# zhipeng-wei/Image-to-Video-I2V-attack

Measured on AMD Instinct MI355X. Metric: adversarial frames/sec (10-step I2V, ResNet-50 layer3, 32x224^2 clips), higher is better.
Workload: dtype f32

## Files before the change

### __graft_entry__.py

```python
import os
import subprocess
import sys

ROOT = os.path.dirname(os.path.abspath(__file__))
PKG_ROOT = os.path.join(ROOT, "image-to-video-i2v-attack_amd")
CSRC = os.path.join(PKG_ROOT, "csrc")
LIB = os.path.join(PKG_ROOT, "i2v_amd", "libi2v_hip.so")
for p in (PKG_ROOT, ROOT):
    if p not in sys.path:
        sys.path.insert(0, p)


def _stale(target, sources):
    return not os.path.exists(target) or any(os.path.getmtime(s) > os.path.getmtime(target) for s in sources)


ENGINE_UNITS = ["i2v_engine.cpp", "i2v_pack.cpp", "i2v_plan.cpp", "i2v_tune.cpp", "i2v_run.cpp", "i2v_loop_api.cpp"]
UNITS = ["i2v_kernels.hip", "i2v_conv_cfg0.hip", "i2v_conv_cfg1.hip", "i2v_conv_cfg2.hip", "i2v_conv_cfg3.hip", "i2v_conv_cfg4.hip",
         "i2v_conv_cfg5.hip", "i2v_conv_scpair.hip", "i2v_conv_stems.hip", "i2v_fastblock.hip", "i2v_gconv.hip", "i2v_dwconv.hip", "i2v_se.hip", "i2v_loader.hip", "i2v_vit.hip", "i2v_vit.cpp", "i2v_swin.hip", "i2v_swin.cpp",
         "i2v_convnext.hip", "i2v_convnext.cpp", "i2v_mixer.hip", "i2v_mixer.cpp",
         ] + ENGINE_UNITS
HEADERS = ["i2v_kernels.h", "i2v_params.h", "i2v_be.h", "i2v_conv_tile.h", "i2v_conv_launch.h", "i2v_vit_kernels.h", "i2v_swin_kernels.h", "i2v_xf.h",
           "i2v_net.h", "i2v_se_host.h", "i2v_convnext_host.h", "i2v_xf_host.h", "i2v_hip_stub.h",
           "i2v_mixer_host.h", "i2v_gelu.h", "i2v_scpair_host.h"]
FLAGS = ["--offload-arch=gfx950", "-O3", "-ffp-contract=off", "-std=c++20", "-fPIC", "-DI2V_SEPARATE_UNITS",
         "-DI2V_HAVE_GCONV", "-DI2V_HAVE_DWCONV",
         "-DI2V_HAVE_SE",
         "-DI2V_HAVE_CONVNEXT",
         "-DI2V_HAVE_MIXER",
         "-DI2V_HAVE_SCPAIR"]


def build_lib(experimental: bool = False) -> str:
    from concurrent.futures import ThreadPoolExecutor
    hipcc = os.environ.get("HIPCC", "/opt/rocm/bin/hipcc")
    lib = LIB.replace(".so", "_exp.so") if experimental else LIB
    objdir = os.path.join(CSRC, "build", "exp" if experimental else "default")
    os.makedirs(objdir, exist_ok=True)
    units = UNITS + (["i2v_conv_exp.hip"] if experimental else [])
    hdrs = [os.path.join(CSRC, f) for f in HEADERS] + [os.path.join(ROOT, "include", h) for h in ("i2v_hip.h", "i2v_loader.h", "i2v_vit.h", "i2v_swin.h", "i2v_convnext.h", "i2v_mixer.h")]
    defs = ["-DI2V_EXPERIMENTAL"] if experimental else []
    if not _stale(lib, [os.path.join(CSRC, u) for u in units] + hdrs):
        return lib
    jobs = []
    for u in units:
        src, obj = os.path.join(CSRC, u), os.path.join(objdir, u + ".o")
        if _stale(obj, [src] + hdrs):
            jobs.append([hipcc] + FLAGS + defs + ["-c", "-x", "hip", src, "-o", obj])

    def run(cmd):
        print(" ".join(cmd), flush=True)
        subprocess.run(cmd, check=True)
    if jobs:
        with ThreadPoolExecutor(max_workers=min(len(jobs), max(1, (os.cpu_count() or 2)))) as ex:
            list(ex.map(run, jobs))
    objs = [os.path.join(objdir, u + ".o") for u in units]
    if jobs or _stale(lib, objs):
        run([hipcc, "--offload-arch=gfx950", "-shared", "-fPIC", "-o", lib] + objs)
    return lib


def build() -> None:
    build_lib(experimental=False)
    deps = [os.path.join(CSRC, f) for f in ENGINE_UNITS + ["i2v_net.h", "i2v_kernels.h", "i2v_params.h", "i2v_se_host.h", "i2v_convnext_host.h", "i2v_convnext.cpp", "i2v_mixer_host.h", "i2v_mixer.cpp", "i2v_scpair_host.h", "i2v_gelu.h", "i2v_xf.h", "i2v_xf_host.h", "i2v_hip_stub.h",
                                                               "i2v_vit_kernels.h", "i2v_swin_kernels.h"]] + [os.path.join(ROOT, "include", "i2v_hip.h")]
    hs = os.path.join(ROOT, "tests", "hostsim")
    if _stale(os.path.join(hs, "libi2v_hostsim.so"), deps + [os.path.join(hs, "hostsim_backend.cpp")]):
        subprocess.run([os.path.join(hs, "build.sh")], check=True)
    import ctypes
    import i2v_amd
    from i2v_amd import lib
    cd = ctypes.CDLL(LIB) if not _has_gpu() else lib.load()
    missing = [n for n in lib.EXPORTS + lib.LOADER_EXPORTS + lib.VIT_EXPORTS + lib.SWIN_EXPORTS + lib.CONVNEXT_EXPORTS + lib.MIXER_EXPORTS if not hasattr(cd, n)]
    if missing:
        raise RuntimeError(f"libi2v_hip.so lacks symbols: {missing}")


def _has_gpu() -> bool:
    try:
        import torch
        return torch.cuda.is_available()
    except Exception:
        return False


def smoke() -> None:
    import numpy as np
    import torch
    build()
    from i2v_amd import attacks, graphs, weights
    from oracle import restate
    gen = torch.Generator().manual_seed(1234)
    u8 = torch.randint(0, 256, (1, 3, 4, 64, 64), generator=gen, dtype=torch.uint8)
    mean = torch.tensor(restate.MEAN).view(1, 3, 1, 1, 1)
    std = torch.tensor(restate.STD).view(1, 3, 1, 1, 1)
    vid = (u8.float() / 255 - mean) / std
    atk = attacks.ImageGuidedFMDirection_Adam(["resnet"], depth=3, step_size=0.005, steps=3,
                                              graph_builder=graphs.build_tiny, weight_seed=0)
    adv = atk(vid, torch.zeros(1, dtype=torch.long), ["smoke"])
    torch.cuda.synchronize()
    g = graphs.build_tiny("resnet", (64, 64))
    net = restate.OracleNet(g, weights.synthetic_state_dict(g, 0), [g.hooks[3]])
    ref = restate.run_attack([net], vid, steps=3, step_size=0.005)
    np.testing.assert_allclose(atk.last_costs, ref["costs"], rtol=2e-4)
    diff = (adv.cpu() - ref["adv"]).abs()
    assert float(diff.mean()) < 5e-3, float(diff.mean())
    print("smoke ok: costs", atk.last_costs, "mean|adv-oracle|", float(diff.mean()))


if __name__ == "__main__":
    if "--experimental" in sys.argv[1:]:
        print(build_lib(experimental=True))
    else:
        build()
        if _has_gpu():
            smoke()
```

### image-to-video-i2v-attack_amd/csrc/i2v_be.h

```cpp
#pragma once
#include <hip/hip_runtime.h>
#include <math.h>
#include <stdint.h>
#include <stdio.h>
#include <stdlib.h>
#include <string.h>

#include <type_traits>
#include <utility>

#include "i2v_kernels.h"

typedef float f32x16 __attribute__((ext_vector_type(16)));
typedef float f32x4 __attribute__((ext_vector_type(4)));

extern thread_local char g_be_err[256];
extern thread_local bool g_be_has_err;
int hip_fail(hipError_t e, const char* what);
#define HIPCHK(x) do { hipError_t e_ = (x); if (e_ != hipSuccess) return hip_fail(e_, #x); } while (0)
#define LAUNCH_CHECK(name) do { hipError_t e_ = hipGetLastError(); if (e_ != hipSuccess) return hip_fail(e_, name); } while (0)
extern long long g_stat_conv, g_stat_pws, g_stat_bf3, g_stat_igh, g_stat_sth, g_stat_fastblock, g_stat_vfma, g_stat_igv, g_stat_gconv, g_stat_dwconv, g_stat_se, g_stat_cndw, g_stat_mixtok, g_stat_scpair;

__device__ __forceinline__ unsigned fastdiv(unsigned n, unsigned m, unsigned s) {
    return (unsigned)(((unsigned long long)n * m) >> s);
}
static inline void fastdiv_magic(unsigned d, uint32_t* m, uint32_t* s) {
    unsigned l = 0; while ((1ull << l) < d) ++l;
    *s = 31 + l;
    *m = (uint32_t)(((1ull << (31 + l)) / d) + 1);
}
typedef int i2v_v4i __attribute__((ext_vector_type(4)));
__device__ __forceinline__ I2VKEntry load_kentry(const I2VKEntry* tab, int k) {
#if defined(__HIP_DEVICE_COMPILE__)
    const i2v_v4i v = ((const __attribute__((address_space(4))) i2v_v4i*)tab)[k];
    return I2VKEntry{v.x, v.y, v.z, v.w};
#else
    return tab[k];
#endif
}

static inline void conv_magics(I2VConvParams& p) {
    fastdiv_magic((unsigned)(p.Hg * p.Wg), &p.dv_hw_m, &p.dv_hw_s);
    fastdiv_magic((unsigned)p.Wg, &p.dv_w_m, &p.dv_w_s);
    fastdiv_magic((unsigned)(p.Tg > 0 ? p.Tg : 1), &p.dv_t_m, &p.dv_t_s);
    fastdiv_magic((unsigned)(p.Wo > 0 ? p.Wo : 1), &p.dv_wo_m, &p.dv_wo_s);
}

static inline bool conv_wants_prefetch(const I2VConvParams& p) {
    return p.vec_epilogue && !p.gate_scale && !p.pre_scale && p.add0_stride == 1 && (p.add0 || p.add1 || p.mask || p.gate) && p.Kpad <= 256 && (p.pointwise || p.tap_uniform) && p.Cd > 32;
}

static inline int conv_tail_px_tiles(const I2VConvParams& p) {
    if (p.quad || p.pre_scale || p.temporal || !(p.pointwise || p.tap_uniform) || p.Cd % 16 != 0 || p.blk > 1) return 0;
    const int64_t P = (int64_t)p.N * p.Hg * p.Wg;
    const int64_t n_px = (P + 63) / 64; const int n_cd = (p.Cd + 63) / 64;
    const int64_t tiles = n_px * n_cd;
    if (tiles < 2 * 256) return 0;
    const int r = (int)(tiles % 256);
    if (r == 0 || r > 104) return 0;
    return r / n_cd;
}

static inline bool conv_halo_ok(const I2VConvParams& p) {
    return p.halo == 9 && p.tap_uniform && !p.temporal && !p.pre_scale && !p.quad && p.blk <= 1 && p.sh == 1 && p.sw == 1 && p.Hs == p.Hg &&
           p.Ws == p.Wg && (p.Ws == 14 || p.Ws == 28 || p.Ws == 56) && p.Kpad == p.K && (p.Kpad / I2V_KC) % 9 == 0;
}

static inline bool conv_dc_ok(const I2VConvParams& p) {
    return (p.pointwise || p.tap_uniform) && !p.temporal && !p.pre_scale && !p.quad && p.Cd > 32 && (p.Kpad / I2V_KC) % 2 == 0 && p.Kpad >= 4 * I2V_KC;
}

static inline bool conv_bf3_ok(const I2VConvParams& p) {
#ifdef I2V_EXPERIMENTAL
    return p.bf3 && p.wp3 && (p.pointwise || p.tap_uniform) && (!p.temporal || p.tap_uniform) && !p.pre_scale && !p.quad && p.blk <= 1 && p.blkt <= 1 && p.Cd > 32;
#else
    (void)p; return false;
#endif
}

int launch_conv_cfg0(const I2VConvParams& p, hipStream_t s);
int launch_conv_cfg1(const I2VConvParams& p, hipStream_t s);
int launch_conv_cfg2(const I2VConvParams& p, hipStream_t s);
int launch_conv_cfg3(const I2VConvParams& p, hipStream_t s);
int launch_conv_cfg4(const I2VConvParams& p, hipStream_t s);
int launch_conv_cfg5(const I2VConvParams& p, hipStream_t s);
bool conv_ighalo_ok(const I2VConvParams& p);
int launch_conv_ighalo(const I2VConvParams& p, hipStream_t s);
bool conv_igvfma_ok(const I2VConvParams& p);
int launch_conv_igvfma(const I2VConvParams& p, hipStream_t s);
bool conv_stemhalo_ok(const I2VConvParams& p);
int launch_conv_stemhalo(const I2VConvParams& p, hipStream_t s);
bool conv_vfma_ok(const I2VConvParams& p);
int launch_conv_vfma(const I2VConvParams& p, hipStream_t s);
#ifdef I2V_EXPERIMENTAL
#ifndef I2V_BF3_VARIANT
#define I2V_BF3_VARIANT 1
#endif
#endif
#ifdef I2V_EXPERIMENTAL
bool conv_stem64_ok(const I2VConvParams& p);
int launch_conv_stem64(const I2VConvParams& p, hipStream_t s);
int conv_pws_grid(const I2VConvParams& p);
int launch_conv_pws(const I2VConvParams& p, hipStream_t s);
int launch_conv_bf3(const I2VConvParams& p, hipStream_t s);
// ... 2 lines not shown
```

### image-to-video-i2v-attack_amd/csrc/i2v_conv_tile.h

```cpp
#pragma once
#include "i2v_be.h"

#ifndef I2V_PROBE_T
struct I2VNoProbe {
    __device__ __forceinline__ void entry() {}
    __device__ __forceinline__ void loop_begin() {}
    __device__ __forceinline__ void loop_end(int ) {}
    __device__ __forceinline__ void exit(int ) {}
};
#define I2V_PROBE_T I2VNoProbe
#endif

#ifndef I2V_PRIO_LEVELS
#define I2V_PRIO_LEVELS 3
#endif
#ifndef I2V_DEEP
#define I2V_DEEP 1
#endif
#ifndef I2V_DEEP_STAGES
#define I2V_DEEP_STAGES 3
#endif
#ifndef I2V_BF3_STAGES
#define I2V_BF3_STAGES 2
#endif
#ifndef I2V_SMALL_WPE
#define I2V_SMALL_WPE 7
#endif
#ifndef I2V_PREF_WPE
#define I2V_PREF_WPE 6
#endif
#ifndef I2V_MID_WPE
#define I2V_MID_WPE 5
#endif
#ifndef I2V_TALL_WPE
#define I2V_TALL_WPE 6
#endif
#ifndef I2V_BIG_WPE
#define I2V_BIG_WPE 3
#endif

static constexpr int conv_waves_per_simd(int BD, int BP, bool PREF, bool hi, int MODE = 0) {
    return (BD == 64 && BP == 64) ? (PREF ? (I2V_DEEP && MODE == 1 && I2V_DEEP_STAGES > 3 ? 4  : I2V_PREF_WPE) : I2V_SMALL_WPE) : (BD == 128 && BP == 64) ? I2V_TALL_WPE : (BD == 32 && BP == 256) ? 4  : BD * BP == 8192 ? I2V_MID_WPE : BD * BP == 16384 ? I2V_BIG_WPE : (hi ? 8 : 1);
}
#define I2V_CONV_WPE __attribute__((amdgpu_waves_per_eu(conv_waves_per_simd(BD, BP, PREF, false, MODE), conv_waves_per_simd(BD, BP, PREF, true, MODE))))
static constexpr bool conv_deep(int MODE, bool PREF) { return I2V_DEEP && PREF && MODE == 1; }
template <int BD, int BP, int WD, bool MF16, int NST = 2, int CPB = 1, int BF3 = 0>
constexpr int conv_lds_floats() {
    constexpr int stage = NST * CPB * (I2V_KC * BP + (BF3 == 2 ? 0 : BF3 ? ((BD / 32) * 3 + 3) / 4 * 4 * 256 : I2V_KC * BD)), epi = WD * (MF16 ? 16 : 32) * BP;
    return stage > epi ? stage : epi;
}

template <int HWM>
constexpr int conv_halo_lds_floats() {
    constexpr int stage = 2 * I2V_KC * (64 + 64 + 2 * HWM + 2), epi = 64 * 64;
    return stage > epi ? stage : epi;
}

template <int BD, int BP, int WD, bool PREF, bool MF16, bool FUSE, typename PT>
__device__ __forceinline__ void conv_vec_rows(const PT& p, const int i, const int cd0, const int64_t px0, const float (*const Cs)[BP], const int t,
                                              const float4* const pre0, const unsigned* const pregw, float* const mid) {
    constexpr int FR = MF16 ? 16 : 32;
    const int lane = t & 63;
    const int HWg = p.Hg * p.Wg, HoWo = p.Ho * p.Wo;
    const int64_t P = (int64_t)p.N * HWg;
    (void)pre0; (void)pregw; (void)mid;
#ifdef I2V_NT_ALL
    const bool nt_store = true;
#else
    const bool nt_store = p.cfg > 0 && ((p.cfg - 1) & 128);
#endif
    constexpr int C4 = BP / 4, RSTEP = 1024 / BP, NQ = WD * FR / RSTEP;
    const int c4 = t % C4, rbase = t / C4;
    const int64_t pp = px0 + (int64_t)c4 * 4;
    const bool pok = pp < P;
    const int64_t n = pok ? fastdiv((unsigned)pp, p.dv_hw_m, p.dv_hw_s) : 0;
    const int64_t poff = pp - n * HWg;
    #pragma unroll
    for (int q = 0; q < NQ; ++q) {
        const int row = rbase + q * RSTEP;
        const int cd = cd0 + (row / FR) * (BD / WD) + i * FR + (row % FR);
        const bool valid = pok && cd < p.Cd;
        float4 v = make_float4(0.f, 0.f, 0.f, 0.f);
        if (valid) {
        v = *reinterpret_cast<const float4*>(&Cs[row][c4 * 4]);
        const int64_t o = (int64_t)cd * HoWo + poff;
        if (p.gate_scale) {
            const float4 m = *reinterpret_cast<const float4*>(p.mask + n * p.mask_nstride + o);
            const float gs = p.gate_scale[cd], gt = p.gate_shift[cd];
            if (!(fmaf(m.x, gs, gt) > 0.f)) v.x = 0.f;
            if (!(fmaf(m.y, gs, gt) > 0.f)) v.y = 0.f;
            if (!(fmaf(m.z, gs, gt) > 0.f)) v.z = 0.f;
            if (!(fmaf(m.w, gs, gt) > 0.f)) v.w = 0.f;
        }
        if (p.shift) { const float sh = p.shift[cd]; v.x += sh; v.y += sh; v.z += sh; v.w += sh; }
        if (PREF) {
            v.x += pre0[q].x; v.y += pre0[q].y; v.z += pre0[q].z; v.w += pre0[q].w;
        } else {
            if (p.add0 && p.add0_stride == 1) {
                const float4 a = *reinterpret_cast<const float4*>(p.add0 + n * p.add0_nstride + o);
                v.x += a.x; v.y += a.y; v.z += a.z; v.w += a.w;
            } else if (p.add0) {
                const int oh = (int)fastdiv((unsigned)poff, p.dv_wo_m, p.dv_wo_s), ow = (int)(poff - (int64_t)oh * p.Wo);
                if (!(oh & 1) && (oh >> 1) < p.add0_H) {
                    const float2 a = *reinterpret_cast<const float2*>(
                        p.add0 + n * p.add0_nstride + (int64_t)cd * p.add0_H * p.add0_W + (oh >> 1) * p.add0_W + (ow >> 1));
                    v.x += a.x; v.z += a.y;
                }
            }
        }
        if (p.add1) {
            const float4 a = *reinterpret_cast<const float4*>(p.add1 + n * p.add1_nstride + o);
            v.x += a.x; v.y += a.y; v.z += a.z; v.w += a.w;
        }
        if (p.relu) { v.x = fmaxf(v.x, 0.f); v.y = fmaxf(v.y, 0.f); v.z = fmaxf(v.z, 0.f); v.w = fmaxf(v.w, 0.f); }
        if (p.gate) {
            const unsigned w = PREF ? pregw[q] : p.gate[(int64_t)cd * p.gate_stride + ((p.gate_pix0 + pp) >> 5)];
            const unsigned g = w >> ((unsigned)(p.gate_pix0 + pp) & 31u);
            if (!(g & 1u)) v.x = 0.f;
            if (!(g & 2u)) v.y = 0.f;
            if (!(g & 4u)) v.z = 0.f;
            if (!(g & 8u)) v.w = 0.f;
        } else if (p.mask && !p.gate_scale) {
            const float4 m = *reinterpret_cast<const float4*>(p.mask + n * p.mask_nstride + o);
            if (!(m.x > 0.f)) v.x = 0.f;
            if (!(m.y > 0.f)) v.y = 0.f;
            if (!(m.z > 0.f)) v.z = 0.f;
            if (!(m.w > 0.f)) v.w = 0.f;
        }
        if constexpr (!FUSE) {
            if (nt_store) { typedef float nt4 __attribute__((ext_vector_type(4))); const nt4 w4 = {v.x, v.y, v.z, v.w};
                            __builtin_nontemporal_store(w4, reinterpret_cast<nt4*>(p.dst + n * p.dst_nstride + o)); }
            else *reinterpret_cast<float4*>(p.dst + n * p.dst_nstride + o) = v;
        }
        }
        if constexpr (FUSE)
            *reinterpret_cast<float4*>(mid + (cd - cd0) * BP + c4 * 4) = v;
        if (p.gate_out) {
            unsigned nib = valid ? ((v.x > 0.f ? 1u : 0u) | (v.y > 0.f ? 2u : 0u) | (v.z > 0.f ? 4u : 0u) | (v.w > 0.f ? 8u : 0u)) : 0u;
            nib <<= 4 * (lane & 7);
            nib |= (unsigned)__builtin_amdgcn_update_dpp(0, (int)nib, 0xB1, 0xF, 0xF, true);
            nib |= (unsigned)__builtin_amdgcn_update_dpp(0, (int)nib, 0x4E, 0xF, 0xF, true);
            nib |= (unsigned)__builtin_amdgcn_update_dpp(0, (int)nib, 0x141, 0xF, 0xF, true);
            if (valid && (lane & 7) == 0)
                p.gate_out[(int64_t)cd * p.gate_out_stride + ((p.gate_out_pix0 + pp) >> 5)] = nib;
        }
    }
}

#define I2V_FROW(r) (MF16 ? 4 * lk + (r) : ((r) & 3) + 8 * ((r) >> 2) + 4 * lk)
template <int BP, int WP, bool MF16, int TP, typename ACC>
__device__ __forceinline__ void conv_acc_to_rows(ACC (&acc)[TP], float (*const Cs)[BP]) {
    constexpr int FR = MF16 ? 16 : 32, NR = MF16 ? 4 : 16;
    const int lane = threadIdx.x & 63, wave = threadIdx.x >> 6;
    const int wd = wave / WP, wpx = wave % WP;
    const int l31 = MF16 ? (lane & 15) : (lane & 31), lk = MF16 ? (lane >> 4) : (lane >> 5);
    __syncthreads();
#pragma unroll
    for (int j = 0; j < TP; ++j)
#pragma unroll
        for (int r = 0; r < NR; ++r)
            Cs[wd * FR + I2V_FROW(r)][wpx * (BP / WP) + j * FR + l31] = acc[j][r];
    __syncthreads();
}
template <int BD, int BP, int WD, int WP, bool PREF, bool MF16, bool FUSE, typename ACC, typename PT>
__device__ __forceinline__ void conv_vec_epilogue(const PT& p, ACC (&acc)[BD / WD / (MF16 ? 16 : 32)][BP / WP / (MF16 ? 16 : 32)], const int cd0,
                                                  const int64_t px0, float* const smem, const float4* const pre0, const unsigned* const pregw,
                                                  float* const mid) {
    constexpr int FR = MF16 ? 16 : 32, TD = BD / WD / FR;
    const int t = threadIdx.x;
    float (*Cs)[BP] = reinterpret_cast<float (*)[BP]>(smem);
#pragma unroll
    for (int i = 0; i < TD; ++i) {
        conv_acc_to_rows<BP, WP, MF16>(acc[i], Cs);
        conv_vec_rows<BD, BP, WD, PREF, MF16, FUSE>(p, i, cd0, px0, Cs, t, pre0, pregw, mid);
    }
}
#undef I2V_FROW

__device__ __forceinline__ int conv_xcd_lid(const int bid, const int nwg) {
    const int q8 = nwg >> 3, r8 = nwg & 7, xcd = bid & 7;
    return (xcd < r8 ? xcd * (q8 + 1) : r8 * (q8 + 1) + (xcd - r8) * q8) + (bid >> 3);
}

template <int BD, int BP, int WD, int WP, int MODE, bool PREF, bool PRE = false, bool VID = false, bool MF16 = false, int HWM = 0, int CPB = 1, int FUSE = 0, int BF3 = 0>
__device__ __forceinline__ void conv_tile_loop(const I2VConvParams& p, const int cd0, const int64_t px0, const int nwg, float* const smem, I2V_PROBE_T& probe,
                                               const int probe_slot, const int prio_arg,
                                               typename std::conditional<MF16, f32x4, f32x16>::type (&acc)[BD / WD / (MF16 ? 16 : 32)][BP / WP / (MF16 ? 16 : 32)],
                                               float4 (&pre0)[PREF ? WD * (MF16 ? 16 : 32) / (1024 / BP) : 1], unsigned (&pregw)[PREF ? WD * (MF16 ? 16 : 32) / (1024 / BP) : 1]) {
#if defined(__HIP_DEVICE_COMPILE__)
    constexpr int KC = I2V_KC;
    constexpr int FR = MF16 ? 16 : 32;
    constexpr int NR = MF16 ? 4 : 16;
    constexpr int TD = BD / WD / FR, TP = BP / WP / FR;
    static_assert(!(MF16 && (PRE || PREF)), "no pre-activation / prefetch variants of the 16x16 tile");
    constexpr bool DEEP = conv_deep(MODE, PREF) || (BF3 == 1 && I2V_BF3_STAGES > 2) || BF3 == 3;
    constexpr int NST = BF3 == 3 ? 3 : BF3 == 1 ? I2V_BF3_STAGES : DEEP ? I2V_DEEP_STAGES : 2, AHEAD = NST - 1;
    constexpr bool HALO = MODE == 5;
    constexpr int HS = HALO ? BP + 2 * HWM + 2 : 1, HQ = (HS + 63) / 64;
    static_assert(!HALO || (HWM > 0 && BD == 64 && BP == 64 && !PREF && !PRE && !VID && !MF16), "halo staging: the plain 64x64 image tile only");
    static_assert(CPB == 1 || (!HALO && !DEEP && !PREF && !PRE && MODE != 4 && MODE != 0), "several chunks per barrier: the plain pointwise / tap-uniform loops only");
    constexpr int KB = CPB * KC;
    static_assert(!BF3 || (!MF16 && !PRE && !PREF && !HALO && (MODE == 1 || MODE == 2) && FUSE == 0 && BD % 32 == 0), "split-bf16 K loop: the plain pointwise / tap-uniform tiles");
    constexpr int AF = BF3 == 2 ? 0 : BF3 ? CPB * (((BD / 32) * 3 + 3) / 4 * 4) * 256 : KB * BD;
    float (*As)[KB][BD] = reinterpret_cast<float (*)[KB][BD]>(smem);
    float* const As3 = smem;
    float (*Bs)[KB][BP] = reinterpret_cast<float (*)[KB][BP]>(smem + NST * AF);

    const int t = threadIdx.x, lane = t & 63, wave = t >> 6;
    const int wd = wave / WP, wpx = wave % WP;

    const int HWg = p.Hg * p.Wg;
    const int64_t P = (int64_t)p.N * HWg;

    constexpr bool PW = MODE == 1;
    constexpr bool QUAD = MODE == 4;
    typedef __attribute__((address_space(3))) void* lds_ptr_t;
    constexpr unsigned OOB = 0x80000000u;
    const int wv = __builtin_amdgcn_readfirstlane(wave);
    const __amdgpu_buffer_rsrc_t rs_w = BF3 ? __builtin_amdgcn_make_buffer_rsrc((void*)p.wp3, 0, (p.Kpad / KC) * (p.Cdpad / 32) * 3072, 0x00020000)
                                            : __builtin_amdgcn_make_buffer_rsrc((void*)p.wp, 0, p.Kpad * p.Cdpad * 4, 0x00020000);
    constexpr unsigned XB = QUAD ? 64u : 0u;
    const __amdgpu_buffer_rsrc_t rs_x = __builtin_amdgcn_make_buffer_rsrc((void*)((const char*)p.src - XB), 0, p.src_span_bytes + 2 * XB, 0x00020000);
    constexpr int NA = BF3 == 2 ? 0 : BF3 ? (BD / 32) * 3 : KC * BD / 256, NAQ = (NA + 3) / 4;
    constexpr int BPER = (PW || QUAD) ? 256 : 64;
    constexpr int NB = HALO ? 0 : KC * BP / BPER, NBQ = (NB + 3) / 4;
    const int bcol = PW ? (lane * 4) % BP : (BP >= 64 ? ((wave * 64) % BP) + lane : lane % BP);
    const int64_t ppix = px0 + bcol;
    const bool pvalid = ppix < P;
    const int64_t pn = pvalid ? fastdiv((unsigned)ppix, p.dv_hw_m, p.dv_hw_s) : 0;
    const int prem = (int)(ppix - pn * HWg);
    const int HWs = p.Hs * p.Ws;
    int h0 = 0, w0 = 0, t0 = 0;
    int64_t pns = pn;
    if (VID) {
        const int64_t clip = fastdiv((unsigned)pn, p.dv_t_m, p.dv_t_s);
        t0 = (int)(pn - clip * p.Tg) * p.st;
        pns = clip * p.Ts + t0;
    }
    const int nstr = (int)p.src_nstride;
    unsigned xoff;
    if (PW) xoff = (unsigned)((pns * p.src_nstride + prem) * 4);
    else {
        const int gi = (int)fastdiv((unsigned)prem, p.dv_w_m, p.dv_w_s), gj = prem - gi * p.Wg;
        h0 = gi * p.sh; w0 = gj * p.sw;
        xoff = (unsigned)((pns * p.src_nstride + (int64_t)h0 * p.Ws + w0) * 4) + XB;
    }
    if (!pvalid) xoff = OOB;
    unsigned aoff[NAQ ? NAQ : 1];
#pragma unroll
    for (int q = 0; q < NAQ; ++q) {
        const int f = (wave + 4 * q) * 256 + lane * 4;
        aoff[q] = BF3 ? (unsigned)(((cd0 / 32) * 3 + wave + 4 * q) * 1024 + lane * 16) : (unsigned)(((f / BD) * p.Cdpad + f % BD + cd0) * 4);
    }
    unsigned boff[PW ? NBQ : 1];
    if (PW) {
#pragma unroll
        for (int q = 0; q < NBQ; ++q) boff[q] = pvalid ? xoff + (unsigned)((((wave + 4 * q) * 256 + lane * 4) / BP) * HWs * 4) : OOB;
// ... 670 lines not shown
```

### image-to-video-i2v-attack_amd/csrc/i2v_engine.cpp

```cpp
#include "i2v_net.h"

#include <math.h>
#include <stdarg.h>
#include <stdio.h>
#include <stdlib.h>
#include <string.h>

using namespace eng;

#define I2V_MAX_NETS 4096
thread_local std::string eng::g_err;

int eng::fail(const char* fmt, ...) {
    char buf[512];
    va_list ap;
    va_start(ap, fmt);
    vsnprintf(buf, sizeof buf, fmt, ap);
    va_end(ap);
    g_err = buf;
    return 1;
}

int i2v_api_fail(const char* msg) { return fail("%s", msg); }

// ... 343 lines not shown
        if (nd.groups > 1 || nd.dw) std::vector<float>().swap(nd.w);
    }
    size_t off = 64;
    for (const Node& nd : n.nodes) if (nd.type == 0 && nd.cd.src == n.input && nd.fwd.quad) n.stage_input = true;
    if (n.stage_input) {
        const Buffer& ib = n.bufs[n.tens[n.input].buf];
        n.in_stage_off = off; off = align_up(off + N * ib.C * ib.H * ib.W, 64) + 64;
    }
    for (Buffer& b : n.bufs) {
        if (b.is_input) continue;
        size_t sz = N / Tin * b.T * b.C * b.H * b.W;
        b.act_off = off; off = align_up(off + sz, 64);
        b.grad_off = off; off = align_up(off + sz, 64);
    }
    const char* gates_env = getenv("I2V_GATES");
    const bool use_gates = !(gates_env && gates_env[0] == '0');
    for (const Node& nd : n.nodes)
        if (use_gates && nd.type == 0 && nd.cd.relu && !nd.fwd.tpair) n.bufs[n.tens[nd.cd.dst].buf].gated = true;
    for (const Node& nd : n.nodes)
        if (use_gates && nd.type == 4 && nd.sd.relu) n.bufs[n.tens[nd.sd.dst].buf].gated = true;
    for (Buffer& b : n.bufs) {
        if (!b.gated) continue;
        const size_t pix = N / Tin * b.T * b.H * b.W;
        if (pix + 64 >= (1ull << 31)) return fail("gate rows of more than 2^31 bits are not supported");
        b.gate_words = (int)((pix + 31) / 32 + 2);
        b.gate_off = off; off = align_up(off + (size_t)b.C * b.gate_words, 64);
    }
    for (Node& nd : n.nodes)
        if (nd.type == 1) {
            const Buffer& db = n.bufs[n.tens[nd.pd.dst].buf];
            nd.idx_off = off; off = align_up(off + (N / Tin * db.T * n.tens[nd.pd.dst].C * db.H * db.W + 3) / 4, 64);
        }
    for (Node& nd : n.nodes)
        if (nd.type == 3) {
            const Buffer& tb = n.bufs[n.tens[nd.ad.theta].buf]; const Buffer& pb = n.bufs[n.tens[nd.ad.phi].buf];
            nd.p_off = off; off = align_up(off + N / Tin * ((size_t)tb.T * tb.H * tb.W) * ((size_t)pb.T * pb.H * pb.W), 64);
        }
    for (Node& nd : n.nodes)
        if (nd.type == 4) {
            const size_t C = (size_t)nd.sd.C, rd = (size_t)nd.sd.rd;
            nd.se_off = off; nd.se_floats = 4 * align_up(N * C, 64) + align_up(N * rd, 64);
            off += nd.se_floats;
        }
    std::string err;
    size_t end = 0;
    if (!plan_pass(n, true, off, N, &end, &err)) return fail("plan: %s", err.c_str());
    n.arena_floats = end + 64;
    n.arena = (float*)be_malloc(n.arena_floats * sizeof(float));
    if (!n.arena) return fail("arena allocation of %zu bytes failed", n.arena_floats * sizeof(float));
    CHECK_BE(be_memset0(n.arena, n.arena_floats * sizeof(float), nullptr));
    if (!plan_pass(n, false, off, N, &end, &err)) return fail("plan: %s", err.c_str());
    mark_fusable(n);
    if (autotune(n)) return 1;
    mark_overlap(n);
    CHECK_BE(be_stream_sync(nullptr));
    n.planned = true;
    return 0;
}

extern "C" int i2v_net_fusion_info(i2v_handle h, int net, int32_t out[4]) {
    Net* n = get_net(h, net); if (!n) return 1;
    if (!n->planned || !out) return fail("i2v_net_fusion_info: net not planned");
    out[0] = out[1] = out[2] = out[3] = 0;
    int k = 0;
    for (const std::vector<Launch>* L : {&n->fwd, &n->bwd}) {
        for (const Launch& l : *L) { out[k] += l.fuse_ok ? 1 : 0; out[2 + k] += (l.fuse_ok && l.fuse_b[0]) ? 1 : 0; }
        ++k;
    }
    return 0;
}

extern "C" int i2v_net_scpair_info(i2v_handle h, int net, int32_t out[4]) {
    Net* n = get_net(h, net); if (!n) return 1;
    if (!n->planned || !out) return fail("i2v_net_scpair_info: net not planned");
    out[0] = out[1] = out[2] = out[3] = 0;
    int k = 0;
    for (const std::vector<Launch>* L : {&n->fwd, &n->bwd}) {
        for (const Launch& l : *L) { out[k] += l.sc_ok ? 1 : 0; out[2 + k] += (l.sc_ok && l.sc_b[0]) ? 1 : 0; }
        ++k;
    }
    return 0;
}

extern "C" size_t i2v_net_workspace_bytes(i2v_handle h, int net) {
    Net* n = get_net(h, net); if (!n) return 0;
    return n->arena_floats * sizeof(float) + n->weight_bytes;
}

#ifndef I2V_SEPARATE_UNITS
#include "i2v_pack.cpp"
#include "i2v_plan.cpp"
#include "i2v_tune.cpp"
#include "i2v_run.cpp"
#include "i2v_loop_api.cpp"
#define fail xf_fail
#include "i2v_convnext.cpp"
#include "i2v_mixer.cpp"
#undef fail
#endif
```

### image-to-video-i2v-attack_amd/csrc/i2v_kernels.h

```cpp
#pragma once
#include <initializer_list>
#include "i2v_params.h"

typedef void* i2v_stream_t;

const char* be_name();
long long be_stat(const char* name);
int  be_set_device(int device);
void* be_malloc(size_t bytes);
void be_free(void* p);
int  be_h2d(void* dst, const void* src, size_t bytes);
int  be_d2d_2d(void* dst, size_t dpitch, const void* src, size_t spitch, size_t width, size_t rows,
               i2v_stream_t s);
int  be_memset0(void* p, size_t bytes, i2v_stream_t s);
const char* be_error();
int  i2v_api_fail(const char* msg);
void* be_event_create();
void be_event_destroy(void* ev);
int  be_event_record(void* ev, i2v_stream_t s);
int  be_event_elapsed_ms(void* start, void* stop, float* ms);
int  be_stream_sync(i2v_stream_t s);
i2v_stream_t be_stream_create();
void be_stream_destroy(i2v_stream_t s);
int  be_stream_wait_event(i2v_stream_t s, void* ev);
int  be_device_sync();

int k_conv(const I2VConvParams& p, i2v_stream_t s);
int k_conv_fusable(const I2VConvParams& a, const I2VConvParams& b);
inline bool i2v_conv_pair_fusable(const I2VConvParams& a, const I2VConvParams& b) {
    if (a.pointwise || !a.tap_uniform || a.temporal || a.quad || a.pre_scale || a.gate_scale || a.blk > 1 || a.blkt > 1) return false;
    for (const I2VConvParams* q : {&a, &b})
        if (!(q->Tg == q->Ts && q->Ts == q->To && q->st == 1 && q->ost == 1 && q->ot0 == 0 && q->blkt <= 1)) return false;
    if (a.sh != 1 || a.sw != 1 || a.Hs != a.Hg || a.Ws != a.Wg || a.Hg != a.Ho || a.Wg != a.Wo || a.osh != 1 || a.osw != 1 || a.oh0 || a.ow0) return false;
    if ((a.Cd != 64 && a.Cd != 128) || a.Kpad != a.K || a.add0_stride > 1) return false;
    if (!b.pointwise || b.temporal || b.quad || b.pre_scale || b.gate_scale || b.blk > 1 || b.blkt > 1 || b.add0_stride > 1) return false;
    if (b.K != a.Cd || b.Kpad != b.K || b.Cs != a.Cd || b.src != a.dst || b.src_nstride != a.dst_nstride) return false;
    if (b.Hs != a.Ho || b.Ws != a.Wo || b.Hg != a.Hg || b.Wg != a.Wg || b.Ho != a.Ho || b.Wo != a.Wo || b.sh != 1 || b.sw != 1 || b.osh != 1 || b.osw != 1 ||
        b.oh0 || b.ow0 || b.Cd < 64 || b.Tg != a.Tg) return false;
    return true;
}
int k_conv_fused(const I2VConvParams& a, const I2VConvParams& b, int halo, i2v_stream_t s);
inline bool i2v_conv_scpair_ok(const I2VConvParams& a, const I2VConvParams& b) {
    for (const I2VConvParams* q : {&a, &b})
        if (q->temporal || q->quad || q->pre_scale || q->gate_scale || q->blk > 1 || q->blkt > 1 || q->bf3) return false;
    if (!(a.pointwise || (a.tap_uniform && a.K == a.Cs && a.Kpad == a.K))) return false;
    if (a.relu || a.mask || a.gate || a.gate_out || a.add0 || a.add1) return false;
    if (a.osh != 1 || a.osw != 1 || a.oh0 || a.ow0 || a.Hg != a.Ho || a.Wg != a.Wo) return false;
    if (!b.pointwise || !b.vec_epilogue) return false;
    if (a.N != b.N || a.Hg != b.Hg || a.Wg != b.Wg || a.Cd != b.Cd || a.Ho != b.Ho || a.Wo != b.Wo) return false;
    return a.dst && b.add0 == a.dst && b.add0_stride == 1 && b.add0_nstride == a.dst_nstride;
}
int k_conv_scpair_ok(const I2VConvParams& a, const I2VConvParams& b);
int k_conv_scpair(const I2VConvParams& a, const I2VConvParams& b, i2v_stream_t s);
int k_conv_candidates(const I2VConvParams& p, int* out);
inline int i2v_fastblock_rows(const I2VConvParams& a, const I2VConvParams& b, const I2VConvParams* c, const I2VConvParams* d) {
    auto plain = [](const I2VConvParams& q) {
        return !q.pre_scale && !q.gate_scale && q.blk <= 1 && q.blkt <= 1 && q.sh == 1 && q.sw == 1 && q.osh == 1 && q.osw == 1 && q.oh0 == 0 &&
               q.ow0 == 0 && q.Hs == q.Hg && q.Hg == q.Ho && q.Ws == q.Wg && q.Wg == q.Wo && q.Tg == q.Ts && q.Ts == q.To && q.st == 1 && q.ost == 1 && q.ot0 == 0 &&
               !q.add1 && !q.mask && q.Kpad % 8 == 0 && q.Kpad <= 512 && q.gate_pix0 == 0 && q.gate_out_pix0 == 0;
    };
    if (!plain(a) || !plain(b) || a.quad || a.add0 || b.add0) return 0;
    const int CM = a.Cd;
    if ((CM != 4 && CM != 8) || b.Cd != CM || b.Cs != CM || b.src != a.dst || b.src_nstride != a.dst_nstride) return 0;
    if (b.Hg != a.Hg || b.Wg != a.Wg || b.Tg != a.Tg || b.N != a.N) return 0;
    const int H = a.Hg, W = a.Wg;
    if ((H * W) % 32 != 0 || (int64_t)a.N * a.src_nstride * 4 >= (1ll << 31)) return 0;
    if (c) {
        if (!plain(*c) || c->quad || !a.relu || !b.relu || a.gate || b.gate || c->gate || !c->relu || !a.shift || !b.shift || !c->shift || !a.gate_out || !b.gate_out || !c->gate_out) return 0;
        if (c->src != b.dst || c->src_nstride != b.dst_nstride || c->Cs != CM || c->K != CM || c->Cd != 4 * CM || c->Hg != H || c->Wg != W || c->Tg != a.Tg || c->N != a.N) return 0;
        if (!c->add0 || c->add0_stride != 1) return 0;
        if (d) {
            if (!plain(*d) || d->quad || d->relu || d->add0 || d->gate || d->gate_out || !d->shift || d->src != a.src || d->src_nstride != a.src_nstride || d->Cs != a.Cs ||
                d->K != a.Cs || d->K != CM || d->Cd != c->Cd || d->Hg != H || d->Wg != W || d->Tg != a.Tg || d->N != a.N || c->add0 != d->dst || c->add0_nstride != d->dst_nstride) return 0;
        }
    } else {
        if (d || a.relu || b.relu || a.gate_out || b.gate_out || a.shift || b.shift || !a.gate || !b.gate || a.K != a.Cs || a.K > 64) return 0;
    }
    int g = W, r32 = 32; while (r32) { const int t = g % r32; g = r32; r32 = t; }
    const int Rq = 32 / g;
    if (H % Rq != 0) return 0;
    int R = Rq;
    while (R * W < 192 && R * 2 <= H && H % (R * 2) == 0) R *= 2;
    if ((size_t)CM * (R + 2) * (W + 2) * 4 > 60 * 1024) return 0;
    return R;
}
int k_fastblock(const I2VConvParams& a, const I2VConvParams& b, const I2VConvParams* c, const I2VConvParams* d, i2v_stream_t s);
int k_gconv_plan(I2VGConvParams* p);
int k_gconv(const I2VGConvParams& p, i2v_stream_t s);
int k_dwconv_plan(I2VDwConvParams* p);
int k_dwconv(const I2VDwConvParams& p, i2v_stream_t s);
int k_se_plan(I2VSeParams* p);
int k_se_squeeze(const I2VSeParams& p, i2v_stream_t s);
int k_se_excite(const I2VSeParams& p, i2v_stream_t s);
int k_se_scale(const I2VSeParams& p, i2v_stream_t s);
int k_convnext_dw_plan(I2VCnDwParams* p);
int k_convnext_dw(const I2VCnDwParams& p, i2v_stream_t s);
int k_mixer_tokens_plan(I2VMixTokParams* p);
int k_mixer_tokens(const I2VMixTokParams& p, i2v_stream_t s);
int k_pool_fwd(const I2VPoolParams& p, i2v_stream_t s);
int k_pool_bwd(const I2VPoolParams& p, i2v_stream_t s);
int k_pool3d_fwd(const I2VPoolParams& p, i2v_stream_t s);
int k_pool3d_bwd(const I2VPoolParams& p, i2v_stream_t s);
int k_avgpool_fwd(const I2VPoolParams& p, i2v_stream_t s);
int k_avgpool_bwd(const I2VPoolParams& p, i2v_stream_t s);
int k_addmask(const I2VAddMaskParams& p, i2v_stream_t s);
int k_cos(const I2VCosParams& p, i2v_stream_t s);
int k_std_reduce(const I2VStdParams& p, i2v_stream_t s);
int k_std_grad(const I2VStdParams& p, i2v_stream_t s);
int k_ilaf_reduce(const I2VIlafParams& p, i2v_stream_t s);
int k_ilaf_grad(const I2VIlafParams& p, i2v_stream_t s);
int k_head_ce(const I2VHeadParams& p, i2v_stream_t s);
int k_clip_from_u8(const uint8_t* frames, float* video, int b, int t, int h, int w, i2v_stream_t s);
int k_clip_resize_crop(const uint8_t* frames, float* video, const int32_t* xtab, const int32_t* ytab, int b, int t, int H, int W,
                       int cy, int cx, int oh, int ow, i2v_stream_t s);
int k_frames_from_video(const float* video, float* x, float* u, int b, int f, int h, int w, i2v_stream_t s);
int k_compose(const float* u, const float* delta, float* x, int b, int f, int h, int w, float eps,
              int video_layout, i2v_stream_t s);
int k_adam(float* delta, float* m, float* v, const float* gx, const float* u, int64_t n, int hw,
           float eps, float step_size, float bc2_sqrt, float w1, float beta2, float w2, float adam_eps,
           i2v_stream_t s);
int k_sign_bim(float* adv, const float* u, const float* grad, int64_t n, int64_t chan_stride,
               float step, float eps, i2v_stream_t s);
int k_sign_delta(float* delta, const float* grad, int64_t n, float step, i2v_stream_t s);
int k_sign_delta_gx(float* delta, const float* gx, const float* u, int64_t n, float eps, float step,
                    i2v_stream_t s);
int k_clip_resample_crop(const uint8_t* frames, float* video, const int32_t* xb, const int32_t* xk, int kx, const int32_t* yb, const int32_t* yk,
                         int ky, int b, int t, int H, int W, int cy, int cx, int oh, int ow, i2v_stream_t s);
int k_tt_grad_mix(const float* grads, float* out, const float* kern , const int* moves , int D, int64_t NC, int T,
                  int HW, float w1, float w, i2v_stream_t s);
int k_attn_gemm(const I2VAttnGemm& p, i2v_stream_t s);
int k_softmax_rows(const I2VSoftmaxRows& p, i2v_stream_t s);
int k_resample_nearest(const float* src, float* dst, int64_t planes, int Hs, int Ws, int Hd, int Wd, const int32_t* map_y,
                       const int32_t* map_x, i2v_stream_t s);
int k_resample_nearest_bwd(const float* g, float* gsrc, int64_t planes, int Hd, int Wd, int Hs, int Ws, const int32_t* ylo,
                           const int32_t* yhi, const int32_t* xlo, const int32_t* xhi, i2v_stream_t s);
int k_grad_post_groups(int b, int c, int f, int h, int w, int mode, int64_t* group_elems);
// ... 12 lines not shown
```

### image-to-video-i2v-attack_amd/csrc/i2v_kernels.hip

```cpp
#include "i2v_be.h"

thread_local char g_be_err[256];
thread_local bool g_be_has_err = false;

int hip_fail(hipError_t e, const char* what) {
    snprintf(g_be_err, sizeof g_be_err, "%s: %s", what, hipGetErrorString(e));
    g_be_has_err = true;
    return 1;
}

const char* be_name() { return "hip:gfx950"; }
long long g_stat_conv = 0, g_stat_pws = 0, g_stat_bf3 = 0, g_stat_igh = 0, g_stat_sth = 0;
long long be_stat(const char* name) {
    if (!strcmp(name, "conv_launches")) return __atomic_load_n(&g_stat_conv, __ATOMIC_RELAXED);
    if (!strcmp(name, "pws_launches")) return __atomic_load_n(&g_stat_pws, __ATOMIC_RELAXED);
    if (!strcmp(name, "bf3_launches")) return __atomic_load_n(&g_stat_bf3, __ATOMIC_RELAXED);
    if (!strcmp(name, "ighalo_launches")) return __atomic_load_n(&g_stat_igh, __ATOMIC_RELAXED);
    if (!strcmp(name, "stemhalo_launches")) return __atomic_load_n(&g_stat_sth, __ATOMIC_RELAXED);
    if (!strcmp(name, "fastblock_launches")) return __atomic_load_n(&g_stat_fastblock, __ATOMIC_RELAXED);
    if (!strcmp(name, "vfma_launches")) return __atomic_load_n(&g_stat_vfma, __ATOMIC_RELAXED);
    if (!strcmp(name, "igvfma_launches")) return __atomic_load_n(&g_stat_igv, __ATOMIC_RELAXED);
    if (!strcmp(name, "gconv_launches")) return __atomic_load_n(&g_stat_gconv, __ATOMIC_RELAXED);
    if (!strcmp(name, "dwconv_launches")) return __atomic_load_n(&g_stat_dwconv, __ATOMIC_RELAXED);
    if (!strcmp(name, "se_launches")) return __atomic_load_n(&g_stat_se, __ATOMIC_RELAXED);
    if (!strcmp(name, "convnext_dw_launches")) return __atomic_load_n(&g_stat_cndw, __ATOMIC_RELAXED);
    if (!strcmp(name, "mixer_tokens_launches")) return __atomic_load_n(&g_stat_mixtok, __ATOMIC_RELAXED);
    if (!strcmp(name, "scpair_launches")) return __atomic_load_n(&g_stat_scpair, __ATOMIC_RELAXED);
#ifdef I2V_EXPERIMENTAL
    if (!strcmp(name, "experimental")) return 1;
#else
    if (!strcmp(name, "experimental")) return 0;
#endif
    return -1;
}
const char* be_error() { return g_be_has_err ? g_be_err : nullptr; }
int be_set_device(int device) { HIPCHK(hipSetDevice(device)); return 0; }
void* be_malloc(size_t bytes) { void* p = nullptr; if (hipMalloc(&p, bytes) != hipSuccess) return nullptr; return p; }
void be_free(void* p) { (void)hipFree(p); }
int be_h2d(void* dst, const void* src, size_t bytes) { HIPCHK(hipMemcpy(dst, src, bytes, hipMemcpyHostToDevice)); return 0; }
int be_d2d_2d(void* dst, size_t dpitch, const void* src, size_t spitch, size_t width, size_t rows, i2v_stream_t s) {
    HIPCHK(hipMemcpy2DAsync(dst, dpitch, src, spitch, width, rows, hipMemcpyDeviceToDevice, (hipStream_t)s));
    return 0;
}
int be_memset0(void* p, size_t bytes, i2v_stream_t s) { HIPCHK(hipMemsetAsync(p, 0, bytes, (hipStream_t)s)); return 0; }

void* be_event_create() { hipEvent_t e = nullptr; if (hipEventCreate(&e) != hipSuccess) return nullptr; return (void*)e; }
void be_event_destroy(void* ev) { (void)hipEventDestroy((hipEvent_t)ev); }
int be_event_record(void* ev, i2v_stream_t s) { HIPCHK(hipEventRecord((hipEvent_t)ev, (hipStream_t)s)); return 0; }
int be_event_elapsed_ms(void* a, void* b, float* ms) { HIPCHK(hipEventElapsedTime(ms, (hipEvent_t)a, (hipEvent_t)b)); return 0; }
int be_stream_sync(i2v_stream_t s) { HIPCHK(hipStreamSynchronize((hipStream_t)s)); return 0; }
int be_device_sync() { HIPCHK(hipDeviceSynchronize()); return 0; }
i2v_stream_t be_stream_create() { hipStream_t s = nullptr; if (hipStreamCreateWithFlags(&s, hipStreamNonBlocking) != hipSuccess) return nullptr; return (i2v_stream_t)s; }
void be_stream_destroy(i2v_stream_t s) { if (s) (void)hipStreamDestroy((hipStream_t)s); }
int be_stream_wait_event(i2v_stream_t s, void* ev) { HIPCHK(hipStreamWaitEvent((hipStream_t)s, (hipEvent_t)ev, 0)); return 0; }

__constant__ float c_mean[3] = {0.485f, 0.456f, 0.406f};
__constant__ float c_std[3] = {0.229f, 0.224f, 0.225f};

static int conv_pick(const I2VConvParams& p) {
    const char* force = getenv("I2V_FORCE_CFG");
    if (force && *force) { const int f = atoi(force); return (p.pre_scale && f != 0 && f != 3) ? 3 : f; }
    if (p.Cd <= 16 && !p.pre_scale) return 5;
    if (conv_bf3_ok(p)) return p.Cd > 64 ? 2 : 3;
    if (conv_wants_prefetch(p)) return 3;
    if (p.pre_scale) {
        const double blocks128 = ceil(p.Cd / 128.0) * ceil((double)p.N * p.Hg * p.Wg / 128.0);
        return (p.Cd > 64 && blocks128 >= 256.0 * 6) ? 0 : 3;
    }
    static const struct { int BD, BP, occ; double ineff; } C[5] = {
        {128, 128, 3, 1.00}, {64, 128, 5, 1.05}, {128, 64, 5, 1.04}, {64, 64, 7, 1.10}, {32, 256, 4, 1.08}};
    const double P = (double)p.N * p.Hg * p.Wg;
    const int nchunks = p.Kpad / I2V_KC;
    int best = 0; double best_t = 1e300;
    for (int i = 0; i < 5; ++i) {
        if (C[i].BD > 32 && p.Cd <= C[i].BD / 2) continue;
        if (C[i].BD == 32 && p.Cd > 32) continue;
        const double blocks = ceil(p.Cd / (double)C[i].BD) * ceil(P / C[i].BP);
        const double rounds = ceil(blocks / 256.0);
        const double fill = blocks / (256.0 * C[i].occ);
        const double mfma = (double)nchunks * (C[i].BD / 32) * (C[i].BP / 32) / 4 * 8 * 64 * C[i].ineff *
                            (1.0 + 0.15 * (fill < 1.0 ? 1.0 - fill : 0.0));
        const double overhead = 1500.0 + (C[i].BD * C[i].BP / 256) * 10.0;
        const double t = rounds * mfma + ceil(rounds / C[i].occ) * overhead;
        if (t < best_t) { best_t = t; best = i; }
    }
    return best;
}

int k_conv_candidates(const I2VConvParams& p, int* out) {
    int n = 0;
    if (p.pre_scale) { if (p.Cd > 64) out[n++] = 0; out[n++] = 3; return n; }
#ifdef I2V_EXPERIMENTAL
    if (conv_bf3_ok(p)) {
        static const int BD3[4] = {128, 64, 128, 64};
        for (int i = 0; i < 4; ++i) {
            if (p.Cd <= BD3[i] / 2) continue;
            out[n++] = i;
            if (I2V_BF3_VARIANT == 2 && (p.Kpad / I2V_KC) % 2 == 0) out[n++] = i | 64;
            if (I2V_BF3_VARIANT == 1 && i == 0 && !p.temporal) out[n++] = 0 | 64;
        }
        return n;
    }
#endif
    static const int BD[5] = {128, 64, 128, 64, 32};
    for (int i = 0; i < 5; ++i) {
        if (BD[i] > 32 && p.Cd <= BD[i] / 2) continue;
        if (BD[i] == 32 && p.Cd > 32) continue;
        out[n++] = i;
    }
    if (conv_wants_prefetch(p)) out[n++] = 3 | 8;
// ... 1306 lines not shown
```

### image-to-video-i2v-attack_amd/csrc/i2v_net.h

```cpp
#pragma once
#include "../../include/i2v_hip.h"
#include "i2v_kernels.h"

#include <stdint.h>

#include <deque>
#include <mutex>
#include <string>
#include <vector>

namespace eng {

#pragma GCC visibility push(hidden)
extern thread_local std::string g_err;
int fail(const char* fmt, ...);
#pragma GCC visibility pop

#define CHECK_BE(expr)                                                            \
    do {                                                                          \
        if ((expr) != 0) return fail("%s: %s", #expr, be_error() ? be_error() : "backend error"); \
    } while (0)

struct Buffer { int C, H, W; int T = 1; size_t act_off = 0, grad_off = 0; bool is_input = false;
                size_t gate_off = 0; int gate_words = 0; bool gated = false; };
struct Tensor { int buf, c_off, C; bool post_relu; float bwd_gain = 1.f; };

struct Packed {
    float* wp = nullptr; I2VKEntry* ktab = nullptr;
    float* wpc = nullptr;
    uint16_t* wp3 = nullptr;
    int K = 0, Kpad = 0, Cd = 0, Cdpad = 0, tap_uniform = 0;
    int halo = 0;
    int ph = 0, pw = 0, Hg = 0, Wg = 0;
    int pt = 0, Tg = 1;
    int has_dt = 0;
    int quad = 0, quad_kw = 0, quad_dw0 = 0;
    int tpair = 0;
    int ig_tt = 0, ig_th = 0, ig_tw = 0;
    int ig_p77 = 0;
};

struct Node {
    int type;
    i2v_se_desc sd{};
    std::vector<float> se_w1, se_b1, se_w2t, se_b2;
    float* se_w1_d = nullptr; float* se_b1_d = nullptr; float* se_w2t_d = nullptr; float* se_b2_d = nullptr;
    size_t se_off = 0, se_floats = 0;
    i2v_attn_desc ad{};
    size_t p_off = 0;
    int src0() const { return type == 0 ? cd.src : type == 3 ? ad.theta : type == 4 ? sd.src : pd.src; }
    int dst0() const { return type == 0 ? cd.dst : type == 3 ? ad.dst : type == 4 ? sd.dst : pd.dst; }
    int residual0() const { return type == 0 ? cd.residual : type == 4 ? sd.residual : -1; }
    i2v_conv3d_desc cd; i2v_pool3d_desc pd;
    std::vector<float> w;
    std::vector<float> shift;
    std::vector<float> pre_scale, pre_shift;
    float* shift_d = nullptr; float* pre_scale_d = nullptr; float* pre_shift_d = nullptr;
    bool preact() const { return !pre_scale.empty(); }
    Packed fwd; std::vector<Packed> bwd;
    int groups = 1; std::vector<float> wg; bool gconv = false;
    float* gw_fwd = nullptr; float* gw_bwd = nullptr; int gw_tapmask[4] = {0, 0, 0, 0};
    int dw = 0; bool dwconv = false;
    struct ImgGrad {
        Packed P; int blk = 0, sh = 1, blkt = 1;
        int ost = 1, ot0 = 0;
        int st = 1, oct = 1; bool skips = false;
        double flop_share = 1.0;
    };
    std::vector<ImgGrad> imgs;
    size_t idx_off = 0;
};

enum Kind { L_CONV, L_IMGGRAD, L_POOLF, L_POOLB, L_ADDMASK, L_AVGF, L_AVGB, L_MEMSET, L_POOL3F, L_POOL3B, L_AGEMM, L_SOFTMAX, L_GCONV, L_DWCONV,
            L_SE_SQUEEZE, L_SE_EXCITE, L_SE_SCALE };
struct Launch {
    Kind kind;
    I2VConvParams conv; I2VPoolParams pool; I2VAddMaskParams am; I2VGConvParams gc; I2VDwConvParams dc; I2VSeParams se;
    I2VAttnGemm ag; I2VSoftmaxRows sm; int sm_rows_per_clip = 0;
    int T = 1;
    bool src_is_input = false;
    bool img_accumulate = false;
    float* ms_ptr = nullptr; size_t ms_floats_per_frame = 0;
    float* se_vec = nullptr; size_t se_vec_floats = 0;
    double se_bytes_per_frame = 0;
    bool ms_gx = false;
    double alg_flops_per_frame = 0;
    int cfg_b[4] = {0, 0, 0, 0};
    int fuse_ok = 0;
    int fuse_b[4] = {0, 0, 0, 0};
    int node = -1;
    int fb_ok = 0;
    int fb_b[4] = {0, 0, 0, 0};
    int sc_ok = 0;
    int sc_b[4] = {0, 0, 0, 0};
    bool sc_private = false;
    int ov_after = -2, ov_join = -1;
};
inline int cfg_bucket(int clips, int max_clips) {
    int b = 0;
    while (b < 3 && (max_clips >> (b + 1)) >= clips && (max_clips >> (b + 1)) >= 1) ++b;
    return b;
}

struct Addend { const float* p; int64_t nstride; int stride, H, W; };

struct Net {
    std::vector<Buffer> bufs; std::vector<Tensor> tens; std::vector<Node> nodes;
    int input = -1; std::vector<int> hooks; int maxN = 0; bool planned = false;
    float* arena = nullptr; size_t arena_floats = 0; std::vector<void*> dev_allocs;
    std::vector<Launch> fwd, bwd;
    int frames = 0;
    int Tin() const { return bufs[tens[input].buf].T; }
    size_t weight_bytes = 0;
    std::vector<float*> hook_tmp;
    size_t in_stage_off = 0; bool stage_input = false;
    i2v_stream_t side = nullptr; std::vector<void*> ov_ev; size_t ov_used = 0;
    std::vector<std::vector<int>> ov_at[2]; int ov_max_frames = 0;
};

struct TimedLaunch { void* start; void* stop; int kind; double flops; int Cd, K, HWg, frames, pw; void* chain_from; double bytes; int count = 1; };

}

struct i2v_ctx {
    int device; std::vector<eng::Net*> nets; std::mutex nets_mu;
    int timing = 0;
    std::deque<eng::TimedLaunch> timed; size_t timed_used = 0; std::mutex timing_mu;
};

namespace eng {
#pragma GCC visibility push(hidden)

inline size_t align_up(size_t v, size_t a) { return (v + a - 1) / a * a; }

inline Net* get_net(i2v_handle h, int id) {
    if (!h || id < 0 || id >= (int)h->nets.size() || !h->nets[id]) { fail("bad net id %d", id); return nullptr; }
    return h->nets[id];
}

template <typename T>
int upload(Net& n, const std::vector<T>& host, T** dev) {
    size_t bytes = host.size() * sizeof(T);
    void* d = be_malloc(bytes ? bytes : 16);
    if (!d) return fail("device allocation of %zu bytes failed", bytes);
    n.dev_allocs.push_back(d);
    n.weight_bytes += bytes;
    if (bytes) CHECK_BE(be_h2d(d, host.data(), bytes));
    *dev = (T*)d;
    return 0;
}

bool math_bf16x3();
int pack_fwd(Net& n, Node& nd);
int pack_bwd(Net& n, Node& nd);
int pack_img(Net& n, Node& nd);
bool gconv_enabled();
int pack_gconv(Net& n, Node& nd);
bool dwconv_enabled();
int pack_dwconv(Net& n, Node& nd);

struct View { float* p; int64_t nstride; int C, H, W; int T = 1; };
View view_of(Net& n, int t, bool grad);
bool plan_pass(Net& n, bool dry, size_t off, size_t N, size_t* end, std::string* err);

void mark_fusable(Net& n);
void mark_overlap(Net& n);
int autotune(Net& n);

I2VConvParams conv_prep(const Launch& l, const float* x, float* gx, int accumulate);
int conv_run(const Launch& l, int frames, const float* x, float* gx, int accumulate, i2v_stream_t s);
bool fused_fits(const Launch& a, const Launch& b, int frames);
int fused_run(const Launch& a, const Launch& b, int frames, const float* x, int halo, i2v_stream_t s);
int fast_run(const std::vector<Launch>& L, size_t li, int frames, const float* x, i2v_stream_t s);
bool sc_pair_ok(const Launch& a, const Launch& b);
bool sc_fits(const Launch& a, const Launch& b, int frames);
int sc_run(const Launch& a, const Launch& b, int frames, i2v_stream_t s);
extern long long g_overlap_launches;

#pragma GCC visibility pop
}
```

### image-to-video-i2v-attack_amd/csrc/i2v_run.cpp

```cpp
#include "i2v_net.h"
#ifndef I2V_HAVE_SE
#include "i2v_se_host.h"
#endif
#ifndef I2V_HAVE_SCPAIR
#include "i2v_scpair_host.h"
#endif

#include <stdio.h>
#include <stdlib.h>

#include <algorithm>

using namespace eng;

namespace eng {

I2VConvParams conv_prep(const Launch& l, const float* x, float* gx, int accumulate) {
    I2VConvParams p = l.conv;
    if (l.src_is_input) p.src = x;
    if (l.kind == L_IMGGRAD) { p.dst = gx; if (accumulate || l.img_accumulate) { p.add1 = gx; p.add1_nstride = p.dst_nstride; } }
    p.vec_epilogue = (p.blk <= 1 && p.osh == 1 && p.osw == 1 && p.oh0 == 0 && p.ow0 == 0 && p.Hg == p.Ho &&
                      p.Wg == p.Wo && p.Tg == p.To && p.ost == 1 && p.ot0 == 0 &&
                      (p.Ho * p.Wo) % 4 == 0 && p.dst_nstride % 4 == 0 &&
                      (p.add0_stride == 1 || (p.add0_stride == 2 && p.Wo % 4 == 0 && p.add0_W * 2 == p.Wo &&
                                              p.add0_W % 2 == 0 && (p.add0_H * p.add0_W) % 2 == 0)) &&
                      p.add0_nstride % 4 == 0 && p.add1_nstride % 4 == 0 && p.mask_nstride % 4 == 0 &&
                      (((uintptr_t)p.dst | (uintptr_t)p.add0 | (uintptr_t)p.add1 | (uintptr_t)p.mask) & 15) == 0)
                         ? 1 : 0;
    if (!(p.Tg == p.Ts && p.Ts == p.To && p.st == 1 && p.ost == 1 && p.ot0 == 0 && p.blkt == 1)) p.temporal = 1;
    return p;
}

bool fused_fits(const Launch& a, const Launch& b, int frames) {
    for (const Launch* l : {&a, &b}) {
        const I2VConvParams& p = l->conv;
        const int64_t span = ((int64_t)frames * p.Ts / p.Tg - 1) * p.src_nstride * 4 + (int64_t)p.Cs * p.Hs * p.Ws * 4;
        if (span >= (1ll << 31)) return false;
    }
    return true;
}
int fused_run(const Launch& a, const Launch& b, int frames, const float* x, int halo, i2v_stream_t s) {
    I2VConvParams pa = conv_prep(a, x, nullptr, 0), pb = conv_prep(b, x, nullptr, 0);
    for (I2VConvParams* p : {&pa, &pb}) {
        p->N = frames;
        p->src_span_bytes = (int32_t)(((int64_t)frames * p->Ts / p->Tg - 1) * p->src_nstride * 4 + (int64_t)p->Cs * p->Hs * p->Ws * 4);
    }
    CHECK_BE(k_conv_fused(pa, pb, halo, s));
    return 0;
}

static void sc_prep(const Launch& a, const Launch& b, int frames, I2VConvParams* pa, I2VConvParams* pb) {
    *pa = conv_prep(a, nullptr, nullptr, 0); *pb = conv_prep(b, nullptr, nullptr, 0);
    for (I2VConvParams* p : {pa, pb}) {
        p->N = frames;
        p->src_span_bytes = (int32_t)(((int64_t)frames * p->Ts / p->Tg - 1) * p->src_nstride * 4 + (int64_t)p->Cs * p->Hs * p->Ws * 4);
    }
}
bool sc_pair_ok(const Launch& a, const Launch& b) {
    if (a.kind != L_CONV || b.kind != L_CONV || a.src_is_input || b.src_is_input || a.T != b.T) return false;
    I2VConvParams pa, pb;
    sc_prep(a, b, a.T, &pa, &pb);
#ifdef I2V_HAVE_SCPAIR
    return k_conv_scpair_ok(pa, pb) != 0;
#else
    return scpair_host::ok(pa, pb) != 0;
#endif
}
bool sc_fits(const Launch& a, const Launch& b, int frames) { return fused_fits(a, b, frames); }
int sc_run(const Launch& a, const Launch& b, int frames, i2v_stream_t s) {
    I2VConvParams pa, pb;
    sc_prep(a, b, frames, &pa, &pb);
#ifdef I2V_HAVE_SCPAIR
    CHECK_BE(k_conv_scpair(pa, pb, s));
#else
    if (scpair_host::run(pa, pb, s)) return fail("shortcut pair: the two launches do not form a pair");
#endif
    return 0;
}

int fast_run(const std::vector<Launch>& L, size_t li, int frames, const float* x, i2v_stream_t s) {
    const int g = L[li].fb_ok;
    I2VConvParams q[4];
    for (int j = 0; j < g; ++j) { q[j] = conv_prep(L[li + j], x, nullptr, 0); q[j].N = frames; }
    const I2VConvParams* c = g == 3 ? &q[2] : g == 4 ? &q[3] : nullptr;
    const I2VConvParams* d = g == 4 ? &q[2] : nullptr;
    if (i2v_fastblock_rows(q[0], q[1], c, d) <= 0) return 2;
    if (k_fastblock(q[0], q[1], c, d, s)) { fail("k_fastblock: %s", be_error() ? be_error() : "backend error"); return 1; }
    return 0;
}

int conv_run(const Launch& l, int frames, const float* x, float* gx, int accumulate, i2v_stream_t s) {
    I2VConvParams p = conv_prep(l, x, gx, accumulate);
    const int clips = frames / p.Tg;
    const int64_t plane_bytes = (int64_t)p.Cs * p.Hs * p.Ws * 4, stride_bytes = p.src_nstride * 4;
    const int64_t clip_bytes = (int64_t)(p.Ts - 1) * stride_bytes + plane_bytes;
    int64_t per = clip_bytes >= (1ll << 31) ? 0 : 1 + ((1ll << 31) - 1 - clip_bytes) / (stride_bytes * p.Ts);
    if (per < 1) return fail("one clip of a convolution input exceeds 2 GiB");
    if (per < clips && (p.gate || p.gate_out)) {
        per -= per % 32;
        if (per < 1) return fail("a sliced convolution launch cannot keep its gate rows word-aligned");
    }
    for (int c0 = 0; c0 < clips; c0 += (int)per) {
        I2VConvParams q = p;
        const int nc = clips - c0 < per ? clips - c0 : (int)per;
        q.N = nc * p.Tg;
        q.src += (int64_t)c0 * p.Ts * p.src_nstride; q.dst += (int64_t)c0 * p.To * p.dst_nstride;
        if (q.add0) q.add0 += (int64_t)c0 * p.To * p.add0_nstride;
        if (q.add1) q.add1 += (int64_t)c0 * p.To * p.add1_nstride;
        if (q.mask) q.mask += (int64_t)c0 * p.To * p.mask_nstride;
        q.gate_pix0 = p.gate_pix0 + (int32_t)((int64_t)c0 * p.To * p.Ho * p.Wo);
        q.gate_out_pix0 = p.gate_out_pix0 + (int32_t)((int64_t)c0 * p.To * p.Ho * p.Wo);
        q.src_span_bytes = (int32_t)((int64_t)(nc * p.Ts - 1) * stride_bytes + plane_bytes);
        CHECK_BE(k_conv(q, s));
    }
    return 0;
}

}

long long eng::g_overlap_launches = 0;

static TimedLaunch* timing_begin(i2v_ctx* h, int kind, double flops, i2v_stream_t s, TimedLaunch* prev) {
    if (!h->timing) return nullptr;
    TimedLaunch* t;
    {
        std::lock_guard<std::mutex> lock(h->timing_mu);
        if (h->timed_used == h->timed.size()) {
            TimedLaunch fresh{be_event_create(), be_event_create(), 0, 0.0, 0, 0, 0, 0, 0, nullptr, 0.0, 1};
            if (!fresh.start || !fresh.stop) return nullptr;
            h->timed.push_back(fresh);
        }
        t = &h->timed[h->timed_used++];
    }
    t->kind = kind; t->flops = flops; t->Cd = t->K = t->HWg = t->frames = t->pw = 0; t->bytes = 0.0; t->count = 1;
    t->chain_from = prev ? prev->stop : nullptr;
    if (!t->chain_from) be_event_record(t->start, s);
    return t;
}

static double launch_flops(const std::vector<Launch>& L, size_t li, int fb, int fuse, int sc, int frames, int clips) {
    const Launch& l = L[li];
    double flops = 0.0;
    if (sc >= 0) return 2.0 * frames * l.conv.Hg * l.conv.Wg * ((double)l.conv.Cd * l.conv.K + (double)L[sc].conv.Cd * L[sc].conv.K);
    if (fb) { for (int j = 0; j < fb; ++j) { const Launch& m = L[li + j]; flops += m.alg_flops_per_frame > 0 ? m.alg_flops_per_frame * frames : 2.0 * frames * m.conv.Hg * m.conv.Wg * (double)m.conv.Cd * m.conv.K; } }
    else if ((l.kind == L_CONV || l.kind == L_GCONV || l.kind == L_DWCONV) && l.alg_flops_per_frame > 0) flops = l.alg_flops_per_frame * frames;
    else if (l.kind == L_CONV) flops = 2.0 * frames * l.conv.Hg * l.conv.Wg * ((double)l.conv.Cd * l.conv.K + (fuse ? (double)L[li + 1].conv.Cd * L[li + 1].conv.K : 0.0));
    else if (l.kind == L_IMGGRAD) flops = l.alg_flops_per_frame * frames;
    else if (l.kind == L_AGEMM) flops = 2.0 * clips * (double)l.ag.Cc * l.ag.M * l.ag.N;
    else if (l.kind == L_SE_SQUEEZE || l.kind == L_SE_EXCITE || l.kind == L_SE_SCALE) flops = l.alg_flops_per_frame * frames;
    return flops;
}

static int launch_timing_kind(const Launch& l, bool backward_pass) {
    switch (l.kind) {
        case L_CONV: case L_AGEMM: case L_GCONV: case L_DWCONV: return backward_pass ? 5 : 0;
        case L_IMGGRAD: return 1;
        case L_POOLF: case L_AVGF: case L_POOL3F: return 2;
        case L_POOLB: case L_AVGB: case L_POOL3B: return 3;
        case L_ADDMASK: case L_MEMSET: case L_SOFTMAX: return 4;
        case L_SE_SQUEEZE: case L_SE_EXCITE: case L_SE_SCALE: return 4;
    }
    return 4;
}

static double launch_bytes(const std::vector<Launch>& L, size_t li, int fb, int fuse, int sc, int frames, int clips, int accumulate) {
    const Launch& l = L[li];
    const I2VConvParams& q = l.conv;
    const double out = (double)frames * q.Hg * q.Wg * q.Cd;
    const double src = (double)clips * q.Ts * q.Cs * q.Hs * q.Ws;
    double b = 4.0 * (src + (double)q.K * q.Cd + out);
    if (q.add0) b += 4.0 * out / (q.add0_stride * q.add0_stride);
    if (q.add1 || l.kind == L_IMGGRAD) b += (q.add1 || accumulate || l.img_accumulate) ? 4.0 * out : 0.0;
    if (q.mask) b += 4.0 * out;
    if (q.gate) b += out / 8.0;
    if (q.gate_out) b += out / 8.0;
    if (fb) {
        const I2VConvParams& last = L[li + fb - 1].conv;
        const double outl = (double)frames * last.Hg * last.Wg * last.Cd;
        b = 4.0 * (src + outl);
        for (int j = 0; j < fb; ++j) {
            const I2VConvParams& r = L[li + j].conv;
            const double o = (double)frames * r.Hg * r.Wg * r.Cd;
            b += 4.0 * (double)r.K * r.Cd + (r.gate ? o / 8.0 : 0.0) + (r.gate_out ? o / 8.0 : 0.0);
        }
        if (fb == 3) b += 4.0 * outl;
    }
    if (fuse) {
        const I2VConvParams& r = L[li + 1].conv;
        const double out2 = (double)frames * r.Hg * r.Wg * r.Cd;
        b += 4.0 * ((double)r.K * r.Cd + out2) - 4.0 * out;
        if (r.add0) b += 4.0 * out2;
        if (r.add1) b += 4.0 * out2;
        if (r.mask) b += 4.0 * out2;
        if (r.gate) b += out2 / 8.0;
        if (r.gate_out) b += out2 / 8.0;
    }
    if (sc >= 0) {
        const I2VConvParams& r = L[sc].conv;
        b += 4.0 * ((double)clips * r.Ts * r.Cs * r.Hs * r.Ws + (double)r.K * r.Cd) - 4.0 * out;
    }
    return b;
}

namespace {

struct ListTiming {
    i2v_ctx* h; i2v_stream_t s; bool backward_pass;
    TimedLaunch* prev = nullptr;
    TimedLaunch* seg = nullptr;

    TimedLaunch* open(const std::vector<Launch>& L, size_t li, int fb, int fuse, int sc, int frames, int clips, int accumulate) {
        const Launch& l = L[li];
        const int kind = launch_timing_kind(l, backward_pass);
        const double flops = launch_flops(L, li, fb, fuse, sc, frames, clips);
        const bool conv = l.kind == L_CONV || l.kind == L_IMGGRAD || l.kind == L_GCONV || l.kind == L_DWCONV;
        if (h->timing == 2) {
            if (!seg || seg->kind != kind) {
                close();
                seg = timing_begin(h, kind, 0.0, s, seg);
                if (seg) seg->count = 0;
            }
            if (seg) { seg->flops += flops; seg->count += 1; if (conv) seg->bytes += launch_bytes(L, li, fb, fuse, sc, frames, clips, accumulate); else seg->bytes += l.se_bytes_per_frame * frames; }
            return prev = nullptr;
        }
        TimedLaunch* const tl = prev = timing_begin(h, kind, flops, s, prev);
        if (tl && conv) {
            tl->Cd = l.conv.Cd; tl->K = l.conv.K; tl->HWg = l.conv.Hg * l.conv.Wg; tl->frames = frames; tl->pw = l.conv.pointwise;
            tl->bytes = launch_bytes(L, li, fb, fuse, sc, frames, clips, accumulate);
        }
        if (tl && l.kind == L_AGEMM) {
            const I2VAttnGemm& q = l.ag;
            tl->Cd = q.Cc; tl->K = q.form == 1 ? q.Cc : (q.form == 2 ? q.N : q.M); tl->HWg = q.form == 2 ? q.M : q.N; tl->frames = frames; tl->pw = 10 + q.form;
            tl->bytes = 4.0 * clips * ((double)q.M * q.N + (double)q.Cc * q.M + (double)q.Cc * q.N);
        }
        if (tl && (l.kind == L_SE_SQUEEZE || l.kind == L_SE_EXCITE || l.kind == L_SE_SCALE)) {
            tl->Cd = l.se.C; tl->K = l.se.rd; tl->HWg = l.se.HW; tl->frames = frames;
            tl->pw = 20 + (l.kind == L_SE_SQUEEZE ? 0 : l.kind == L_SE_EXCITE ? 1 : 2) + 3 * l.se.backward;
            tl->bytes = l.se_bytes_per_frame * frames;
        }
        return tl;
    }
    void close() { if (seg) be_event_record(seg->stop, s); }
};

struct SideStream {
    Net& n; std::vector<Launch>& L; const std::vector<std::vector<int>>& at; i2v_stream_t main;
    int clips; const float* x; float* gx; int accumulate;
    struct Pending { int join; void* done; };
    std::vector<Pending> pending;

    void* event() {
        if (n.ov_used == n.ov_ev.size()) { void* e = be_event_create(); if (!e) return nullptr; n.ov_ev.push_back(e); }
        return n.ov_ev[n.ov_used++];
    }
    int issue(int p) {
        for (int i : at[p + 1]) {
            void* ready = event(); void* done = event();
            if (!ready || !done) return fail("launch overlap: event creation failed");
            CHECK_BE(be_event_record(ready, main)); CHECK_BE(be_stream_wait_event(n.side, ready));
            Launch& m = L[i];
            const int fr = clips * m.T;
            if (fr * m.conv.Hg * m.conv.Wg != 0) {
                const int cb = m.cfg_b[cfg_bucket(clips, n.maxN / n.Tin())];
                if (cb) m.conv.cfg = cb;
                if (conv_run(m, fr, x, gx, accumulate, n.side)) return 1;
                __atomic_fetch_add(&g_overlap_launches, 1, __ATOMIC_RELAXED);
            }
            CHECK_BE(be_event_record(done, n.side));
            pending.push_back(Pending{m.ov_join, done});
        }
        return 0;
    }
    int join(int upto) {
        for (size_t i = 0; i < pending.size();) {
            if (pending[i].join <= upto) { CHECK_BE(be_stream_wait_event(main, pending[i].done)); pending[i] = pending.back(); pending.pop_back(); }
            else ++i;
        }
        return 0;
    }
};

}

static int run_list(i2v_ctx* h, Net& n, std::vector<Launch>& L, int in_frames, const float* x, float* gx, int accumulate,
                    i2v_stream_t s, bool backward_pass) {
    const int clips = in_frames / n.Tin();
    const int bucket = cfg_bucket(clips, n.maxN / n.Tin());
    ListTiming timing{h, s, backward_pass};
    SideStream side{n, L, n.ov_at[backward_pass ? 1 : 0], s, clips, x, gx, accumulate};
    const bool overlap = !h->timing && n.side && !side.at.empty() && in_frames <= n.ov_max_frames;
    if (overlap) n.ov_used = 0;
    if (overlap && side.issue(-1)) return 1;
    auto leads_group = [&](size_t k) { return L[k].kind == L_CONV && ((L[k].fuse_ok && L[k].fuse_b[bucket]) || (L[k].fb_ok && L[k].fb_b[bucket])); };
    int sc_from = -1; size_t sc_at = 0;
    for (size_t li = 0; li < L.size(); ++li) {
        Launch& l = L[li];
        const int frames = clips * l.T;
        const size_t li0 = li;
        if (overlap && l.ov_after != -2) continue;
        if (l.kind == L_CONV && l.sc_ok && l.sc_b[bucket] && !overlap && sc_from < 0 && li + l.sc_ok < L.size() && frames * l.conv.Hg * l.conv.Wg > 0 &&
            sc_fits(l, L[li + l.sc_ok], frames)) {
            bool clear = !leads_group(li);
            for (size_t k = li + 1; k <= li + l.sc_ok && clear; ++k) clear = !leads_group(k);
            if (clear) { sc_from = (int)li; sc_at = li + l.sc_ok; continue; }
        }
        const int sc = (sc_from >= 0 && li == sc_at) ? sc_from : -1;
        if (sc >= 0) sc_from = -1;
        const int fuse = (l.kind == L_CONV && l.fuse_ok && li + 1 < L.size() && frames * l.conv.Hg * l.conv.Wg > 0 && fused_fits(l, L[li + 1], frames))
                             ? l.fuse_b[bucket] : 0;
        const int fb = (l.kind == L_CONV && l.fb_ok && li + l.fb_ok <= L.size() && frames * l.conv.Hg * l.conv.Wg > 0) ? l.fb_b[bucket] * l.fb_ok : 0;
        if (overlap && side.join((int)li + (fb ? fb - 1 : fuse ? 1 : 0))) return 1;
        TimedLaunch* const tl = h->timing ? timing.open(L, li, fb, fuse, sc, frames, clips, accumulate) : nullptr;
        struct Stop { TimedLaunch* t; i2v_stream_t s; ~Stop() { if (t) be_event_record(t->stop, s); } } stop{tl, s};
        switch (l.kind) {
            case L_CONV:
            case L_IMGGRAD: {
                if (frames * l.conv.Hg * l.conv.Wg == 0) break;
                if (sc >= 0) {
                    if (l.cfg_b[bucket]) l.conv.cfg = l.cfg_b[bucket];
                    if (sc_run(L[sc], l, frames, s)) return 1;
                    break;
                }
                if (fuse) { if (fused_run(l, L[li + 1], frames, x, fuse == 2, s)) return 1; ++li; break; }
                if (fb) {
                    const int rc = fast_run(L, li, frames, x, s);
                    if (rc == 1) return 1;
                    if (rc == 0) { li += fb - 1; break; }
                }
                const int cb = l.cfg_b[bucket];
                if (cb) l.conv.cfg = cb;
                if (conv_run(l, frames, x, gx, accumulate, s)) return 1;
            } break;
            case L_GCONV: {
#ifdef I2V_HAVE_GCONV
                I2VGConvParams p = l.gc; p.N = frames; CHECK_BE(k_gconv(p, s));
#else
                return fail("this build has no grouped-convolution kernel");
#endif
            } break;
            case L_DWCONV: {
#ifdef I2V_HAVE_DWCONV
                I2VDwConvParams p = l.dc; p.N = frames; CHECK_BE(k_dwconv(p, s));
#else
                return fail("this build has no depthwise-convolution kernel");
#endif
            } break;
#ifdef I2V_HAVE_SE
            case L_SE_SQUEEZE: { I2VSeParams p = l.se; p.N = frames; CHECK_BE(k_se_squeeze(p, s)); } break;
            case L_SE_EXCITE: { I2VSeParams p = l.se; p.N = frames; CHECK_BE(k_se_excite(p, s)); } break;
            case L_SE_SCALE: { I2VSeParams p = l.se; p.N = frames; CHECK_BE(k_se_scale(p, s)); } break;
#else
            case L_SE_SQUEEZE: { I2VSeParams p = l.se; p.N = frames; if (se_host::squeeze(p)) return fail("squeeze-and-excitation: squeeze failed"); } break;
            case L_SE_EXCITE: { I2VSeParams p = l.se; p.N = frames; if (se_host::excite(p)) return fail("squeeze-and-excitation: excite failed"); } break;
            case L_SE_SCALE: { I2VSeParams p = l.se; p.N = frames; if (se_host::scale(p)) return fail("squeeze-and-excitation: scale failed"); } break;
#endif
            case L_POOLF: { I2VPoolParams p = l.pool; p.N = frames; CHECK_BE(k_pool_fwd(p, s)); } break;
            case L_POOL3F: {
                I2VPoolParams p = l.pool; p.N = frames;
                if (p.kt == 1 && p.pad_t == 0 && p.Ts == p.stride_t * p.To) { p.x_nstride *= p.stride_t; CHECK_BE(k_pool_fwd(p, s)); }
                else CHECK_BE(k_pool3d_fwd(p, s));
            } break;
            case L_POOL3B: {
                I2VPoolParams p = l.pool; p.N = frames;
                if (p.kt == 1 && p.pad_t == 0 && p.Ts == p.stride_t * p.To && p.gx_nstride == (int64_t)p.C * p.Hs * p.Ws) {
                    CHECK_BE(be_memset0(p.gx, (size_t)frames * p.stride_t * p.gx_nstride * sizeof(float), s));
                    p.x_nstride *= p.stride_t; p.gx_nstride *= p.stride_t;
                    CHECK_BE(k_pool_bwd(p, s));
                } else CHECK_BE(k_pool3d_bwd(p, s));
            } break;
            case L_AVGF: { I2VPoolParams p = l.pool; p.N = frames; CHECK_BE(k_avgpool_fwd(p, s)); } break;
            case L_AVGB: { I2VPoolParams p = l.pool; p.N = frames; CHECK_BE(k_avgpool_bwd(p, s)); } break;
            case L_MEMSET:
                if (!l.ms_gx) CHECK_BE(be_memset0(l.ms_ptr, l.ms_floats_per_frame * frames * sizeof(float), s));
                else if (!accumulate) CHECK_BE(be_memset0(gx, l.ms_floats_per_frame * frames * sizeof(float), s));
                break;
            case L_POOLB: { I2VPoolParams p = l.pool; p.N = frames; CHECK_BE(k_pool_bwd(p, s)); } break;
            case L_ADDMASK: { I2VAddMaskParams p = l.am; p.N = frames; CHECK_BE(k_addmask(p, s)); } break;
            case L_AGEMM: { I2VAttnGemm p = l.ag; p.clips = clips; CHECK_BE(k_attn_gemm(p, s)); } break;
            case L_SOFTMAX: { I2VSoftmaxRows p = l.sm; p.rows = (int64_t)clips * l.sm_rows_per_clip; CHECK_BE(k_softmax_rows(p, s)); } break;
        }
        if (overlap) for (size_t p = li0; p <= li; ++p) if (side.issue((int)p)) return 1;
    }
    if (overlap && side.join((int)L.size())) return 1;
    timing.close();
    return 0;
}

extern "C" int i2v_net_forward(i2v_handle h, int net, const float* x, int frames, void* stream) {
    Net* n = get_net(h, net); if (!n) return 1;
    if (!n->planned) return fail("net not planned");
    if (frames <= 0 || frames > n->maxN) return fail("frames=%d outside 1..%d", frames, n->maxN);
    if (frames % n->Tin()) return fail("frames=%d is not a multiple of the input's %d frames per clip", frames, n->Tin());
    if (!x) return fail("null input");
    n->frames = frames;
    if (n->stage_input) {
        static const bool always = [] { const char* e = getenv("I2V_STAGE_COPY"); return e && e[0] == '1'; }();
        bool need = always || ((uintptr_t)x & 15) != 0;
        const int bucket = cfg_bucket(frames / n->Tin(), n->maxN / n->Tin());
        for (const Launch& l : n->fwd)
            if (l.kind == L_CONV && l.src_is_input && l.conv.quad && !(l.cfg_b[bucket] > 0 && ((l.cfg_b[bucket] - 1) & 1024))) need = true;
        if (need) {
            const Buffer& ib = n->bufs[n->tens[n->input].buf];
            const size_t bytes = (size_t)frames * ib.C * ib.H * ib.W * sizeof(float);
            float* staged = n->arena + n->in_stage_off;
            CHECK_BE(be_d2d_2d(staged, bytes, x, bytes, bytes, 1, stream));
            x = staged;
// ... 115 lines not shown
```

### image-to-video-i2v-attack_amd/csrc/i2v_tune.cpp

```cpp
#include "i2v_net.h"

#include <stdio.h>
#include <stdlib.h>
#include <string.h>

#include <algorithm>

namespace eng {

void mark_fusable(Net& n) {
    const int64_t frames = n.maxN, clips = n.maxN / n.Tin();
    typedef std::pair<const float*, const float*> Range;
    auto rng = [](const void* q, int64_t fr, int64_t ns, int64_t plane) {
        const float* f = (const float*)q;
        return f ? Range(f, f + (fr > 0 ? (fr - 1) * ns : 0) + std::max<int64_t>(plane, 1)) : Range(nullptr, nullptr);
    };
    auto meet = [](const Range& a, const Range& b) { return a.first && b.first && a.first < b.second && b.first < a.second; };
    auto touches = [&](const Launch& c, const Range& w, bool skip_src, bool skip_dst) {
        if (c.kind == L_CONV || c.kind == L_IMGGRAD || c.kind == L_GCONV || c.kind == L_DWCONV) {
            const I2VConvParams& q = c.conv;
            const int64_t fs = clips * std::max(1, q.Ts), fo = clips * std::max(1, q.To), dplane = (int64_t)(q.blk > 1 ? q.Cd / (q.blk * q.blk) : q.Cd) * q.Ho * q.Wo;
            return (!skip_src && meet(w, rng(q.src, fs, q.src_nstride, (int64_t)q.Cs * q.Hs * q.Ws))) ||
                   meet(w, rng(q.add0, fo, q.add0_nstride, dplane)) || meet(w, rng(q.add1, fo, q.add1_nstride, dplane)) ||
                   meet(w, rng(q.mask, fo, q.mask_nstride, dplane)) || (!skip_dst && meet(w, rng(q.dst, fo, q.dst_nstride, dplane)));
// ... 80 lines not shown
            const I2VConvParams& px = x.conv;
            const bool dep = touches(x, dst_of(a), false, false) || touches(a, dst_of(x), false, false) || touches(x, dst_of(b), false, false) || touches(b, dst_of(x), false, false) ||
                             (px.gate_out && (px.gate_out == a.conv.gate || px.gate_out == b.conv.gate));
            if (!dep) { Launch t = x; n.bwd[i + 1] = n.bwd[i]; n.bwd[i] = t; }
        }
        for (size_t i = 0; !fb_off && i + 1 < n.bwd.size(); ++i) {
            Launch& a = n.bwd[i]; Launch& b = n.bwd[i + 1];
            const i2v_conv3d_desc* ca = cd_of(a); const i2v_conv3d_desc* cb = cd_of(b);
            if (!ca || !cb || !is_pw(*ca) || !is_33(*cb) || a.T != b.T || b.conv.src != a.conv.dst) continue;
            if (i2v_fastblock_rows(a.conv, b.conv, nullptr, nullptr) <= 0) continue;
            if (!private_to(&n.bwd, i, i + 1, a)) continue;
            a.fb_ok = 2;
        }
        for (size_t i = 0; !fb_off && i + 2 < n.fwd.size(); ++i) {
            Launch& a = n.fwd[i]; Launch& b = n.fwd[i + 1];
            const i2v_conv3d_desc* ca = cd_of(a); const i2v_conv3d_desc* cb = cd_of(b);
            if (!ca || !cb || a.src_is_input || !(is_t(*ca) || is_pw(*ca)) || !is_33(*cb) || !ca->relu || !cb->relu || ca->residual >= 0 || cb->residual >= 0 || cb->src != ca->dst) continue;
            Launch& c3 = n.fwd[i + 2];
            const i2v_conv3d_desc* cc = cd_of(c3);
            if (!cc || !is_pw(*cc)) continue;
            if (cc->src == cb->dst && cc->residual >= 0 && cc->relu && a.T == b.T && a.T == c3.T) {
                if (i2v_fastblock_rows(a.conv, b.conv, &c3.conv, nullptr) <= 0) continue;
                if (!private_to(&n.fwd, i, i + 2, a) || !private_to(&n.fwd, i, i + 2, b)) continue;
                a.fb_ok = 3;
            } else if (i + 3 < n.fwd.size() && cc->src == ca->src && !cc->relu && cc->residual < 0) {
                Launch& c4 = n.fwd[i + 3];
                const i2v_conv3d_desc* c4d = cd_of(c4);
                if (!c4d || !is_pw(*c4d) || c4d->src != cb->dst || c4d->residual != cc->dst || !c4d->relu || a.T != b.T || a.T != c3.T || a.T != c4.T) continue;
                if (i2v_fastblock_rows(a.conv, b.conv, &c4.conv, &c3.conv) <= 0) continue;
                if (!private_to(&n.fwd, i, i + 3, a) || !private_to(&n.fwd, i, i + 3, b) || !private_to(&n.fwd, i, i + 3, c3)) continue;
                a.fb_ok = 4;
            }
        }
        const bool fb_force = [] { const char* e = getenv("I2V_FORCE_FASTBLOCK"); return e && e[0] == '1'; }();
        for (std::vector<Launch>* L : {&n.fwd, &n.bwd})
            for (Launch& a : *L)
                for (int bk = 0; bk < 4; ++bk) a.fb_b[bk] = (a.fb_ok && fb_force) ? 1 : 0;
        if (getenv("I2V_FUSE_DEBUG"))
            for (std::vector<Launch>* L : {&n.fwd, &n.bwd})
                for (size_t i = 0; i < L->size(); ++i)
                    if ((*L)[i].fb_ok) fprintf(stderr, "[i2v fastblock] %s launch %zu: group of %d (Cs %d -> %d mid channels, %dx%d)\n", L == &n.fwd ? "fwd" : "bwd", i, (*L)[i].fb_ok,
                                               (*L)[i].conv.Cs, (*L)[i].conv.Cd, (*L)[i].conv.Hg, (*L)[i].conv.Wg);
    }
    {
        const bool sc_off = [] { const char* e = getenv("I2V_SCPAIR"); return e && e[0] == '0'; }();
        for (std::vector<Launch>* L : {&n.fwd, &n.bwd}) {
            for (Launch& l : *L) { l.sc_ok = 0; l.sc_private = false; for (int bk = 0; bk < 4; ++bk) l.sc_b[bk] = 0; }
            for (size_t i = 0; !sc_off && i + 1 < L->size(); ++i) {
                Launch& a = (*L)[i];
                if (a.kind != L_CONV || a.src_is_input || a.conv.add0 || a.conv.relu) continue;
                for (size_t j = i + 1; j < L->size() && j <= i + 3; ++j) {
                    const Launch& b = (*L)[j];
                    if (b.kind != L_CONV || b.conv.add0 != a.conv.dst) continue;
                    if (!sc_pair_ok(a, b)) break;
                    const Range w = dst_of(a);
                    auto conv_kind = [](const Launch& c) { return c.kind == L_CONV || c.kind == L_IMGGRAD || c.kind == L_GCONV || c.kind == L_DWCONV; };
                    auto reads = [&](const Launch& c) { return touches(c, w, false, conv_kind(c)); };
                    auto covers = [&](const Launch& c) { return conv_kind(c) && c.conv.dst && dst_of(c).first <= w.first && dst_of(c).second >= w.second; };
                    Launch b_rest = b; b_rest.conv.add0 = nullptr;
                    bool other = reads(b_rest), dead = covers(b);
                    for (size_t k = i + 1; k < j && !other; ++k) other |= touches((*L)[k], w, false, false);
                    for (size_t k = j + 1; k < L->size() && !other && !dead; ++k) {
                        if (reads((*L)[k])) other = true;
                        else if (covers((*L)[k])) dead = true;
                        else other = touches((*L)[k], w, false, false);
                    }
                    if (!dead) {
                        for (auto& hk : hooked) other |= meet(hk, w);
                        for (const Launch& c : (L == &n.fwd ? n.bwd : n.fwd)) other = other || touches(c, w, false, false);
                    }
                    bool dep = false;
                    for (size_t k = i + 1; k < j && !dep; ++k) {
                        const Launch& m = (*L)[k];
                        const I2VConvParams& pa = a.conv; const I2VConvParams& pm = m.conv;
                        dep = (m.kind != L_CONV && m.kind != L_GCONV && m.kind != L_DWCONV) || m.src_is_input || touches(a, dst_of(m), false, false) ||
                              (pm.gate_out && (pm.gate_out == pa.gate || pm.gate_out == pa.gate_out)) || (pa.gate_out && (pa.gate_out == pm.gate || pa.gate_out == pm.gate_out));
                    }
                    if (!other && !dep) { a.sc_ok = (int)(j - i); a.sc_private = !dead; for (int bk = 0; bk < 4; ++bk) a.sc_b[bk] = 1; }
                    if (getenv("I2V_FUSE_DEBUG"))
                        fprintf(stderr, "[i2v scpair] %s launches %zu + %zu (K %d + %d -> Cd %d, %dx%d): other_reader=%d dependent=%d\n", L == &n.fwd ? "fwd" : "bwd", i, j,
                                a.conv.K, b.conv.K, b.conv.Cd, b.conv.Hg, b.conv.Wg, (int)other, (int)dep);
                    break;
                }
            }
        }
    }
    const char* force = getenv("I2V_FORCE_FUSE");
    const int f = force ? atoi(force) : 0;
    for (std::vector<Launch>* L : {&n.fwd, &n.bwd})
        for (Launch& a : *L)
            for (int b = 0; b < 4; ++b) a.fuse_b[b] = (a.fuse_ok && f) ? ((f == 2 && (a.fuse_ok & 2)) ? 2 : 1) : 0;
}

void mark_overlap(Net& n) {
    for (int k = 0; k < 2; ++k) n.ov_at[k].clear();
    for (std::vector<Launch>* L : {&n.fwd, &n.bwd}) for (Launch& l : *L) { l.ov_after = -2; l.ov_join = -1; }
    const char* e = getenv("I2V_OVERLAP_MAX_FRAMES");
    n.ov_max_frames = e ? atoi(e) : 0;
    if (n.ov_max_frames <= 0) return;
    const int64_t clips = n.maxN / n.Tin();
    typedef std::pair<const char*, const char*> Range;
    struct RW { std::vector<Range> r, w; bool barrier = false; };
    static const char gx_tag[16] = {0};
    const Range GX(gx_tag, gx_tag + 16);
    auto rng = [](const void* q, int64_t fr, int64_t stride_bytes, int64_t plane_bytes) {
        const char* f = (const char*)q;
        return f ? Range(f, f + (fr > 0 ? (fr - 1) * stride_bytes : 0) + std::max<int64_t>(plane_bytes, 1)) : Range(nullptr, nullptr);
    };
    auto rw_of = [&](const Launch& c) {
        RW o;
        auto rd = [&](const Range& x) { if (x.first) o.r.push_back(x); };
        auto wr = [&](const Range& x) { if (x.first) o.w.push_back(x); };
        if (c.kind == L_CONV || c.kind == L_IMGGRAD || c.kind == L_GCONV || c.kind == L_DWCONV) {
            const I2VConvParams& q = c.conv;
            const int64_t fs = clips * std::max(1, q.Ts), fo = clips * std::max(1, q.To);
            const int64_t dplane = 4ll * (q.blk > 1 ? q.Cd / (q.blk * q.blk) : q.Cd) * q.Ho * q.Wo;
            if (!c.src_is_input) rd(rng(q.src, fs, 4 * q.src_nstride, 4ll * q.Cs * q.Hs * q.Ws));
            rd(rng(q.add0, fo, 4 * q.add0_nstride, dplane)); rd(rng(q.add1, fo, 4 * q.add1_nstride, dplane)); rd(rng(q.mask, fo, 4 * q.mask_nstride, dplane));
            rd(rng(q.gate, 1, 0, 4ll * q.Cd * q.gate_stride)); wr(rng(q.gate_out, 1, 0, 4ll * q.Cd * q.gate_out_stride));
            if (c.kind == L_IMGGRAD) { wr(GX); rd(GX); } else wr(rng(q.dst, fo, 4 * q.dst_nstride, dplane));
        } else if (c.kind == L_ADDMASK) {
            const int64_t fr = clips * std::max(1, c.T), pl = 4ll * c.am.C * c.am.HW;
            wr(rng(c.am.out, fr, 4 * c.am.out_nstride, pl));
            for (int i = 0; i < 3; ++i) rd(rng(c.am.a[i], fr, 4 * c.am.a_nstride[i], pl));
            rd(rng(c.am.mask, fr, 4 * c.am.mask_nstride, pl)); rd(rng(c.am.gate, 1, 0, 4ll * c.am.C * c.am.gate_stride));
        } else if (c.kind == L_MEMSET) {
            if (c.ms_gx) wr(GX); else wr(rng(c.ms_ptr, 1, 0, 4ll * (int64_t)c.ms_floats_per_frame * clips * std::max(1, c.T)));
        } else if (c.kind == L_AGEMM || c.kind == L_SOFTMAX) {
            o.barrier = true;
        } else if (c.kind == L_SE_SQUEEZE || c.kind == L_SE_EXCITE || c.kind == L_SE_SCALE) {
            const I2VSeParams& q = c.se;
            const int64_t fr = clips * std::max(1, c.T), pl = 4ll * q.C * q.HW;
            const Range vec = rng(c.se_vec, 1, 0, 4ll * (int64_t)c.se_vec_floats);
            rd(vec); wr(vec);
            if (c.kind != L_SE_EXCITE) { rd(rng(q.x, fr, 4 * q.x_nstride, pl)); rd(rng(q.g, fr, 4 * q.g_nstride, pl)); }
            if (c.kind == L_SE_SCALE) {
                rd(rng(q.r, fr, 4 * q.r_nstride, pl)); wr(rng(q.dst, fr, 4 * q.dst_nstride, pl));
                wr(rng(q.gate_out, 1, 0, 4ll * q.C * q.gate_out_stride));
            }
        } else {
            const I2VPoolParams& q = c.pool;
            const int64_t fr = clips * std::max(std::max(1, c.T), std::max(q.Ts, q.To)), pin = 4ll * q.C * q.Hs * q.Ws, pout = 4ll * q.C * q.Ho * q.Wo;
            const Range idx = rng(q.idx, 1, 0, fr * (int64_t)q.C * q.Ho * q.Wo);
            const bool fwd = c.kind == L_POOLF || c.kind == L_POOL3F || c.kind == L_AVGF;
            if (fwd) { rd(rng(q.x, fr, 4 * q.x_nstride, pin)); wr(rng(q.y, fr, 4 * q.y_nstride, pout)); wr(idx); }
            else { rd(rng(q.x, fr, 4 * q.x_nstride, pin)); rd(rng(q.y, fr, 4 * q.y_nstride, pout)); rd(rng(q.yact, fr, 4 * q.yact_nstride, pout)); rd(idx);
                   wr(rng(q.gx, fr * std::max(1, q.stride_t), 4 * q.gx_nstride, pin)); }
        }
        return o;
    };
    auto meet = [](const std::vector<Range>& A, const std::vector<Range>& B) {
        for (const Range& a : A) for (const Range& b : B) if (a.first < b.second && b.first < a.second) return true;
        return false;
    };
    auto conflict = [&](const RW& a, const RW& b) { return a.barrier || b.barrier || meet(a.r, b.w) || meet(a.w, b.w) || meet(a.w, b.r); };
    int k = 0;
    for (std::vector<Launch>* L : {&n.fwd, &n.bwd}) {
        const int M = (int)L->size();
        std::vector<RW> rw; rw.reserve(M);
        for (const Launch& l : *L) rw.push_back(rw_of(l));
        std::vector<char> member(M, 0);
        for (int i = 0; i < M; ++i) {
            const Launch& l = (*L)[i];
            for (int j = 0; j < l.fb_ok && i + j < M; ++j) member[i + j] = 1;
            if (l.fuse_ok) { member[i] = 1; if (i + 1 < M) member[i + 1] = 1; }
        }
        n.ov_at[k].assign(M + 1, {});
        int hoisted = 0;
        for (int i = 1; i < M; ++i) {
            Launch& l = (*L)[i];
            if (l.kind != L_CONV || member[i] || l.src_is_input) continue;
            int dep = -1;
            for (int j = i - 1; j >= 0; --j) if (conflict(rw[i], rw[j])) { dep = j; break; }
            if (dep >= i - 1) continue;
            if (dep >= 0 && (*L)[dep].ov_after != -2) continue;
            int join = M;
            for (int j = i + 1; j < M; ++j) if (conflict(rw[j], rw[i])) { join = j; break; }
            l.ov_after = dep; l.ov_join = join;
            n.ov_at[k][dep + 1].push_back(i);
            ++hoisted;
            if (getenv("I2V_FUSE_DEBUG"))
                fprintf(stderr, "[i2v overlap] %s launch %d (Cd %d, K %d, %dx%d): side stream after launch %d, joined before launch %d of %d\n", k ? "bwd" : "fwd", i,
                        l.conv.Cd, l.conv.K, l.conv.Hg, l.conv.Wg, dep, join, M);
        }
        if (!hoisted) n.ov_at[k].clear();
        ++k;
    }
    if (n.ov_at[0].empty() && n.ov_at[1].empty()) return;
    n.side = be_stream_create();
    if (!n.side) { n.ov_at[0].clear(); n.ov_at[1].clear(); }
}

namespace {

struct Probe {
    float* scratch = nullptr; void* e0 = nullptr; void* e1 = nullptr;
    const float* x = nullptr; float* gx = nullptr;

    int init(Net& n) {
        const Buffer& ib = n.bufs[n.tens[n.input].buf];
        const size_t img = (size_t)n.maxN * ib.C * ib.H * ib.W;
        scratch = (float*)be_malloc(2 * img * sizeof(float));
        if (!scratch) return fail("autotune scratch allocation failed");
        CHECK_BE(be_memset0(scratch, 2 * img * sizeof(float), nullptr));
        e0 = be_event_create(); e1 = be_event_create();
        x = n.stage_input ? n.arena + n.in_stage_off : scratch;
        gx = scratch + img;
        return 0;
    }
    ~Probe() { if (e0) be_event_destroy(e0); if (e1) be_event_destroy(e1); if (scratch) be_free(scratch); }

    template <class F>
    int time(F&& fn, int reps, float* ms_per_run, bool warm_up = true) {
        if (warm_up && fn()) return 1;
        be_event_record(e0, nullptr);
        for (int r = 0; r < reps; ++r) if (fn()) return 1;
        be_event_record(e1, nullptr);
        if (be_stream_sync(nullptr)) return 1;
        float ms = 0.f; be_event_elapsed_ms(e0, e1, &ms);
        *ms_per_run = ms / reps;
        return 0;
    }
};

template <class F>
int for_each_bucket(int max_clips, int Tg, F&& fn) {
    for (int b = 3; b >= 0; --b) {
        const int clips_b = max_clips >> b;
        if (clips_b < 1 || (b > 0 && clips_b == (max_clips >> (b - 1)))) continue;
        if (const int rc = fn(b, clips_b * Tg)) return rc;
    }
    return 0;
}

const char* list_name(const Net& n, const std::vector<Launch>* L) { return L == &n.fwd ? "fwd" : "bwd"; }

int tune_tiles(Net& n, Probe& pr, int max_clips) {
    for (std::vector<Launch>* L : {&n.fwd, &n.bwd})
        for (Launch& l : *L) {
            if (l.kind != L_CONV && l.kind != L_IMGGRAD) continue;
            const int planned_cfg = l.conv.cfg;
            const int reps = l.kind == L_IMGGRAD ? 4 : 2;
            const int rc = for_each_bucket(max_clips, l.conv.Tg, [&](int b, int lf) -> int {
                if (lf * l.conv.Hg * l.conv.Wg == 0) return 0;
                int cand[16]; I2VConvParams probe = l.conv; probe.N = lf;
                probe.temporal = conv_prep(l, pr.x, pr.gx, 0).temporal;
                const int nc = k_conv_candidates(probe, cand);
                if (nc <= 1) { if (nc == 1) l.cfg_b[b] = cand[0] + 1; return 0; }
// ... 32 lines not shown
            Launch& a = (*L)[i];
            if (!a.fb_ok || i + a.fb_ok > L->size()) continue;
            for (int bk = 0; bk < 4; ++bk) a.fb_b[bk] = 0;
            const int rc = for_each_bucket(max_clips, a.conv.Tg, [&](int bk, int lf) -> int {
                auto run_sep = [&]() { for (int j = 0; j < a.fb_ok; ++j) { Launch& m = (*L)[i + j]; if (m.cfg_b[bk]) m.conv.cfg = m.cfg_b[bk]; if (conv_run(m, lf, pr.x, pr.gx, 0, nullptr)) return 1; } return 0; };
                auto run_fb = [&]() { return fast_run(*L, i, lf, pr.x, nullptr); };
                float t_sep = 0.f, t_fb = 0.f;
                if (run_fb() != 0) return 0;
                if (pr.time(run_sep, 3, &t_sep) || pr.time(run_fb, 3, &t_fb)) return 1;
                a.fb_b[bk] = (fb_force || t_fb < 0.97f * t_sep) ? 1 : 0;
                if (getenv("I2V_FUSE_DEBUG"))
                    fprintf(stderr, "[i2v fastblock] %s group %zu (%d launches, %d -> %d mid channels) at %d frames: separate %.1f us, fused %.1f us -> %s\n",
                            list_name(n, L), i, a.fb_ok, a.conv.Cs, a.conv.Cd, lf, 1e3f * t_sep, 1e3f * t_fb, a.fb_b[bk] ? "fused" : "separate");
                return 0;
            });
            for (int j = 0; j < a.fb_ok; ++j) { Launch& m = (*L)[i + j]; m.conv.cfg = m.cfg_b[0] ? m.cfg_b[0] : m.conv.cfg; }
            if (rc) return 1;
        }
    return 0;
}

int tune_pairs(Net& n, Probe& pr, int max_clips) {
    for (std::vector<Launch>* L : {&n.fwd, &n.bwd})
        for (size_t i = 0; i + 1 < L->size(); ++i) {
            Launch& a = (*L)[i]; Launch& b = (*L)[i + 1];
            if (!a.fuse_ok) continue;
            for (int bk = 0; bk < 4; ++bk) a.fuse_b[bk] = 0;
            const int rc = for_each_bucket(max_clips, a.conv.Tg, [&](int bk, int lf) -> int {
                if (!fused_fits(a, b, lf)) return 0;
                const int ca = a.conv.cfg, cb = b.conv.cfg;
                if (a.cfg_b[bk]) a.conv.cfg = a.cfg_b[bk];
                if (b.cfg_b[bk]) b.conv.cfg = b.cfg_b[bk];
                float best = 1e30f; int best_v = 0, rc = 0;
                for (int v = 0; v <= ((a.fuse_ok & 2) ? 2 : 1); ++v) {
                    auto once = [&]() { return v == 0 ? (conv_run(a, lf, pr.x, pr.gx, 0, nullptr) || conv_run(b, lf, pr.x, pr.gx, 0, nullptr))
                                                      : fused_run(a, b, lf, pr.x, v == 2, nullptr); };
                    if (v > 0 && once()) {
                        if (getenv("I2V_FUSE_DEBUG")) fprintf(stderr, "[i2v fuse] pair %zu variant %d does not launch: %s\n", i, v, g_err.c_str());
                        g_err.clear(); continue;
                    }
                    float ms = 0.f;
                    if (pr.time(once, 2, &ms, v == 0)) { rc = 1; break; }
                    if ((v == 0 ? ms : ms * 1.03f) < best) { best = v == 0 ? ms : ms * 1.03f; best_v = v; }
                    if (getenv("I2V_FUSE_DEBUG"))
                        fprintf(stderr, "[i2v fuse] %s pair %zu (Cd %d -> %d, %dx%d) at %d frames: variant %d = %.1f us\n", list_name(n, L), i,
                                a.conv.Cd, b.conv.Cd, a.conv.Hg, a.conv.Wg, lf, v, 1e3f * ms);
                }
                a.fuse_b[bk] = best_v;
                a.conv.cfg = ca; b.conv.cfg = cb;
                return rc;
            });
            if (rc) return 1;
        }
    return 0;
}

int tune_scpairs(Net& n, Probe& pr, int max_clips) {
    for (std::vector<Launch>* L : {&n.fwd, &n.bwd})
        for (size_t i = 0; i < L->size(); ++i) {
            Launch& a = (*L)[i];
            if (!a.sc_ok || i + a.sc_ok >= L->size()) continue;
            Launch& b = (*L)[i + a.sc_ok];
            const int rc = for_each_bucket(max_clips, a.conv.Tg, [&](int bk, int lf) -> int {
                if (lf * a.conv.Hg * a.conv.Wg == 0 || !sc_fits(a, b, lf)) return 0;
                const int ca = a.conv.cfg, cb = b.conv.cfg;
                if (a.cfg_b[bk]) a.conv.cfg = a.cfg_b[bk];
                if (b.cfg_b[bk]) b.conv.cfg = b.cfg_b[bk];
                float t_sep = 0.f, t_pair = 0.f;
                const int rc = pr.time([&] { return conv_run(a, lf, pr.x, pr.gx, 0, nullptr) || conv_run(b, lf, pr.x, pr.gx, 0, nullptr); }, 3, &t_sep) ||
                               pr.time([&] { return sc_run(a, b, lf, nullptr); }, 3, &t_pair);
                a.conv.cfg = ca; b.conv.cfg = cb;
                if (rc) return 1;
                a.sc_b[bk] = t_pair < t_sep ? 1 : 0;
                if (getenv("I2V_FUSE_DEBUG"))
                    fprintf(stderr, "[i2v scpair] %s launches %zu + %zu (K %d + %d -> Cd %d, %dx%d) at %d frames: separate %.1f us, pair %.1f us -> %s\n", list_name(n, L), i,
                            i + a.sc_ok, a.conv.K, b.conv.K, b.conv.Cd, b.conv.Hg, b.conv.Wg, lf, 1e3f * t_sep, 1e3f * t_pair, a.sc_b[bk] ? "pair" : "separate");
                return 0;
            });
            if (rc) return 1;
        }
    return 0;
}

}

int autotune(Net& n) {
    const char* off = getenv("I2V_AUTOTUNE");
    if (off && off[0] == '0') return 0;
    int rc;
    {
        Probe pr;
        if (pr.init(n)) return 1;
        const int max_clips = n.maxN / n.Tin();
        const bool on_device = strncmp(be_name(), "hip", 3) == 0;
        rc = tune_tiles(n, pr, max_clips);
        if (!rc && on_device) rc = tune_fastblocks(n, pr, max_clips);
        if (!rc && on_device) rc = tune_scpairs(n, pr, max_clips);
        static const bool fuse_on = [] { const char* e = getenv("I2V_FUSE"); return e && e[0] == '1'; }();
        if (!rc && fuse_on && on_device) rc = tune_pairs(n, pr, max_clips);
    }
    if (rc) return g_err.empty() ? fail("autotune failed") : 1;
    CHECK_BE(be_memset0(n.arena, n.arena_floats * sizeof(float), nullptr));
    return 0;
}

}
```

### image-to-video-i2v-attack_amd/i2v_amd/engine.py

```python
import ctypes as C
import sys
import threading
import time
from typing import List, Sequence

import torch

from . import lib as _lib
from .graphs import ConvNextSpec, Graph, MixerSpec, SwinSpec, VitSpec
from .weights import fold_affine, fold_pre_affine


_DEVICE_TYPES = {}


def _ptr(t: torch.Tensor, eng: "Engine" = None):
    assert t.is_contiguous() and t.dtype == torch.float32, (t.dtype, t.is_contiguous())
    ok = t.device.type == eng.device.type if eng is not None else _DEVICE_TYPES.get(t.device.type, 0) > 0
    if not ok:
        where = eng.device if eng is not None else sorted(k for k, v in _DEVICE_TYPES.items() if v > 0)
        raise _lib.I2VError(f"tensor on {t.device} passed to an engine on {where}: move it to the engine's device")
    return C.c_void_p(t.data_ptr())


# ... 317 lines not shown
                    d = _lib.Conv3dDesc(self.ten_id[nd.src], self.ten_id[nd.dst], nd.cin, nd.cout, nd.kt, nd.kh, nd.kw,
                                        nd.stride_t, nd.stride, nd.pad_t, nd.pad, nd.dil_t, 1 if nd.relu else 0,
                                        -1 if nd.residual is None else self.ten_id[nd.residual])
                    _lib.check(capi, capi.i2v_net_add_conv3d(h, self.id, C.byref(d), _hptr(w), _hptr(scale), _hptr(shift)))
                    continue
                d = _lib.ConvDesc(self.ten_id[nd.src], self.ten_id[nd.dst], nd.cin, nd.cout, nd.kh, nd.kw,
                                  nd.stride, nd.pad, 1 if nd.relu else 0,
                                  -1 if nd.residual is None else self.ten_id[nd.residual])
                if nd.pre_bn:
                    ps, pt = fold_pre_affine(nd, sd)
                    ps, pt = ps.contiguous(), pt.contiguous()
                    _lib.check(capi, capi.i2v_net_add_conv_preact(h, self.id, C.byref(d), _hptr(w), _hptr(scale), _hptr(shift),
                                                                  _hptr(ps), _hptr(pt)))
                elif getattr(nd, "groups", 1) > 1 and nd.groups == nd.cin == nd.cout:
                    _lib.check(capi, capi.i2v_net_add_conv_depthwise(h, self.id, C.byref(d), _hptr(w), _hptr(scale), _hptr(shift)))
                elif getattr(nd, "groups", 1) > 1:
                    _lib.check(capi, capi.i2v_net_add_conv_grouped(h, self.id, C.byref(d), nd.groups, _hptr(w), _hptr(scale), _hptr(shift)))
                else:
                    _lib.check(capi, capi.i2v_net_add_conv(h, self.id, C.byref(d), _hptr(w), _hptr(scale), _hptr(shift)))
            elif nd.op == "se":
                w1 = sd[nd.fc1 + ".weight"].float().cpu().reshape(nd.rd, nd.C).contiguous()
                w2 = sd[nd.fc2 + ".weight"].float().cpu().reshape(nd.C, nd.rd).contiguous()
                b1, b2 = sd[nd.fc1 + ".bias"].float().cpu().contiguous(), sd[nd.fc2 + ".bias"].float().cpu().contiguous()
                d = _lib.SeDesc(self.ten_id[nd.src], self.ten_id[nd.dst], -1 if nd.residual is None else self.ten_id[nd.residual],
                                nd.C, nd.rd, 1 if nd.relu else 0)
                _lib.check(capi, capi.i2v_net_add_se(h, self.id, C.byref(d), _hptr(w1), _hptr(b1), _hptr(w2), _hptr(b2)))
            elif nd.op == "attention":
                d = _lib.AttnDesc(self.ten_id[nd.src], self.ten_id[nd.phi], self.ten_id[nd.g], self.ten_id[nd.dst], float(nd.scale))
                _lib.check(capi, capi.i2v_net_add_attention(h, self.id, C.byref(d)))
            elif g.video:
                d = _lib.Pool3dDesc(self.ten_id[nd.src], self.ten_id[nd.dst], nd.kt, nd.k, nd.stride_t, nd.stride, nd.pad_t, nd.pad)
                _lib.check(capi, capi.i2v_net_add_maxpool3d(h, self.id, C.byref(d)))
            else:
                d = _lib.PoolDesc(self.ten_id[nd.src], self.ten_id[nd.dst], nd.k, nd.stride, nd.pad)
                add = capi.i2v_net_add_avgpool if nd.op == "avgpool" else capi.i2v_net_add_maxpool
                _lib.check(capi, add(h, self.id, C.byref(d)))
        for t, gain in (relu_gain or {}).items():
            if t in self.ten_id:
                _lib.check(capi, capi.i2v_net_set_relu_gain(h, self.id, self.ten_id[t], float(gain)))
        hooks = (C.c_int * len(hook_tensors))(*[self.ten_id[t] for t in hook_tensors])
        _lib.check(capi, capi.i2v_net_plan(h, self.id, hooks, len(hook_tensors), max_frames))
        self.hook_tensors = hook_tensors
        self.hooks = [self._hook_info(i) for i in range(len(hook_tensors))]

    def _hook_info(self, i) -> HookInfo:
        act, grad = C.c_void_p(), C.c_void_p()
        a_s, g_s, D, pr = C.c_int64(), C.c_int64(), C.c_int64(), C.c_int32()
        _lib.check(self.eng.capi, self.eng.capi.i2v_net_hook_info(
            self.eng.h, self.id, i, C.byref(act), C.byref(a_s), C.byref(grad), C.byref(g_s), C.byref(D), C.byref(pr)))
        hi = HookInfo()
        hi.act, hi.act_stride, hi.grad, hi.grad_stride = act.value, a_s.value, grad.value, g_s.value
        hi.D, hi.post_relu = D.value, pr.value
        ts = self.graph.tensors[self.hook_tensors[i]]
        hi.shape = (ts.C, ts.H, ts.W)
        hi.T = ts.T
        return hi

    def close(self):
        if self.id is not None and self.eng.h:
            with self.eng.plan_lock:
                self.eng.capi.i2v_net_destroy(self.eng.h, self.id)
        self.id = None

    def __del__(self):
        try:
            if not sys.is_finalizing():
                self.close()
        except Exception:
            pass

    def workspace_bytes(self) -> int:
        return self.eng.capi.i2v_net_workspace_bytes(self.eng.h, self.id)

    def fusion_info(self):
        out = (C.c_int32 * 4)()
        _lib.check(self.eng.capi, self.eng.capi.i2v_net_fusion_info(self.eng.h, self.id, out))
        return tuple(int(v) for v in out)

    def scpair_info(self):
        out = (C.c_int32 * 4)()
        _lib.check(self.eng.capi, self.eng.capi.i2v_net_scpair_info(self.eng.h, self.id, out))
        return tuple(int(v) for v in out)

    def forward(self, x: torch.Tensor):
        _lib.check(self.eng.capi, self.eng.capi.i2v_net_forward(self.eng.h, self.id, _ptr(x, self.eng), x.shape[0], self.eng.stream()))

    def backward(self, gx: torch.Tensor, accumulate=False):
        _lib.check(self.eng.capi, self.eng.capi.i2v_net_backward(self.eng.h, self.id, _ptr(gx, self.eng), 1 if accumulate else 0,
                                                                 self.eng.stream()))

    def read_tensor(self, tid: int, frames: int, grad=False) -> torch.Tensor:
        ts = self.graph.tensors[tid]
        out = torch.empty(frames, ts.C, ts.H, ts.W, dtype=torch.float32, device=self.eng.device)
        _lib.check(self.eng.capi, self.eng.capi.i2v_net_read_tensor(self.eng.h, self.id, self.ten_id[tid], 1 if grad else 0,
                                                                    _ptr(out, self.eng), frames, self.eng.stream()))
        return out

    def save_hook(self, i: int, frames: int) -> torch.Tensor:
        return self.read_tensor(self.hook_tensors[i], frames)

    def cossim(self, i: int, init: torch.Tensor, cos_out: torch.Tensor, scratch: torch.Tensor, frames: int,
               coef_dev=None, coef_index=0, coef_host=1.0):
        hi = self.hooks[i]
        capi = self.eng.capi
        _lib.check(capi, capi.i2v_cossim_fwd_bwd_f32(
            C.c_void_p(hi.act), hi.act_stride, _ptr(init, self.eng), hi.D, hi.D, frames,
            C.c_void_p(coef_dev.data_ptr()) if coef_dev is not None else C.c_void_p(0), coef_index, coef_host,
            hi.post_relu, 0, C.c_void_p(cos_out.data_ptr()), C.c_void_p(hi.grad), hi.grad_stride,
            C.c_void_p(scratch.data_ptr()), self.eng.stream()))

    def stdloss(self, i: int, std_out: torch.Tensor, scratch: torch.Tensor, frames: int, exchange=None):
        hi = self.hooks[i]
        capi = self.eng.capi
        _lib.check(capi, capi.i2v_std_reduce_f32(C.c_void_p(hi.act), hi.act_stride, hi.D, frames,
                                                 C.c_void_p(scratch.data_ptr()), self.eng.stream()))
        total = frames * hi.D
        if exchange is not None:
            total = exchange(scratch[:16].view(torch.float64), total)
        _lib.check(capi, capi.i2v_std_grad_f32(
            C.c_void_p(hi.act), hi.act_stride, hi.D, frames, total, hi.post_relu, 0, C.c_void_p(std_out.data_ptr()),
            C.c_void_p(hi.grad), hi.grad_stride, C.c_void_p(scratch.data_ptr()), self.eng.stream()))

    def hook_frames(self, i: int, in_frames: int) -> int:
        return in_frames // self.graph.tensors[self.graph.input].T * self.hooks[i].T

    def ilaf_scratch_bytes(self, i: int, frames: int, frames_per_seg: int = 0) -> int:
        return self.eng.capi.i2v_ilaf_scratch_bytes(self.hooks[i].D, frames, frames_per_seg)

    def ilaf_reduce(self, i: int, ori: torch.Tensor, adv0: torch.Tensor, scratch: torch.Tensor, frames: int, act=None,
                    frames_per_seg: int = 0):
        hi = self.hooks[i]
        capi = self.eng.capi
        a, a_s = (C.c_void_p(hi.act), hi.act_stride) if act is None else (_ptr(act, self.eng), hi.D)
        if frames_per_seg:
            _lib.check(capi, capi.i2v_ilaf_reduce_seg_f32(a, a_s, _ptr(ori, self.eng), _ptr(adv0, self.eng), hi.D, frames, frames_per_seg,
                                                          C.c_void_p(scratch.data_ptr()), self.eng.stream()))
            return
        _lib.check(capi, capi.i2v_ilaf_reduce_f32(a, a_s, _ptr(ori, self.eng), _ptr(adv0, self.eng), hi.D, frames,
                                                  C.c_void_p(scratch.data_ptr()), self.eng.stream()))

    def ilaf_grad(self, i: int, ori, adv0, init_norm, loss_out: torch.Tensor, scratch: torch.Tensor, frames: int,
                  frames_per_seg: int = 0):
        hi = self.hooks[i]
        capi = self.eng.capi
        if frames_per_seg:
            assert init_norm.dtype == torch.float64 and init_norm.numel() == frames // frames_per_seg
            _lib.check(capi, capi.i2v_ilaf_grad_seg_f32(C.c_void_p(hi.act), hi.act_stride, _ptr(ori, self.eng), _ptr(adv0, self.eng), hi.D, frames,
                                                        frames_per_seg, C.c_void_p(init_norm.data_ptr()), hi.post_relu, 0,
                                                        C.c_void_p(loss_out.data_ptr()), C.c_void_p(hi.grad), hi.grad_stride,
                                                        C.c_void_p(scratch.data_ptr()), self.eng.stream()))
            return
        _lib.check(capi, capi.i2v_ilaf_grad_f32(C.c_void_p(hi.act), hi.act_stride, _ptr(ori, self.eng), _ptr(adv0, self.eng), hi.D, frames,
                                                init_norm, hi.post_relu, 0, C.c_void_p(loss_out.data_ptr()),
                                                C.c_void_p(hi.grad), hi.grad_stride, C.c_void_p(scratch.data_ptr()),
                                                self.eng.stream()))

    def tap_distance(self, i: int, clean: torch.Tensor, coef: float, dist_out: torch.Tensor, scratch: torch.Tensor, frames: int,
                     frames_per_seg: int):
        hi = self.hooks[i]
        _lib.check(self.eng.capi, self.eng.capi.i2v_tap_distance_f32(
            C.c_void_p(hi.act), hi.act_stride, _ptr(clean, self.eng), hi.D, frames, frames_per_seg, float(coef), hi.post_relu, 0,
            C.c_void_p(dist_out.data_ptr()), C.c_void_p(hi.grad), hi.grad_stride, C.c_void_p(scratch.data_ptr()), self.eng.stream()))

    def head_ce(self, i, W: torch.Tensor, bias, labels: torch.Tensor, in_frames: int, scale: float, logits: torch.Tensor,
                loss_each: torch.Tensor, scratch: torch.Tensor):
        capi = self.eng.capi
# ... 185 lines not shown
```

### image-to-video-i2v-attack_amd/i2v_amd/lib.py

```python
import ctypes as C
import os

_HERE = os.path.dirname(os.path.abspath(__file__))
LIB_PATH = os.path.join(_HERE, "libi2v_hip.so")
HIP_BACKEND = b"hip:gfx950"


class ConvDesc(C.Structure):
    _fields_ = [(n, C.c_int32) for n in
                ("src", "dst", "cin", "cout", "kh", "kw", "stride", "pad", "relu", "residual")]


class PoolDesc(C.Structure):
    _fields_ = [(n, C.c_int32) for n in ("src", "dst", "k", "stride", "pad")]


class Conv3dDesc(C.Structure):
    _fields_ = [(n, C.c_int32) for n in
                ("src", "dst", "cin", "cout", "kt", "kh", "kw", "stride_t", "stride", "pad_t", "pad", "dil_t",
                 "relu", "residual")]


class AttnDesc(C.Structure):
    _fields_ = [(n, C.c_int32) for n in ("theta", "phi", "g", "dst")] + [("scale", C.c_float)]


class SeDesc(C.Structure):
    _fields_ = [(n, C.c_int32) for n in ("src", "dst", "residual", "C", "rd", "relu")]


class Pool3dDesc(C.Structure):
    _fields_ = [(n, C.c_int32) for n in ("src", "dst", "kt", "k", "stride_t", "stride", "pad_t", "pad")]


class I2VError(RuntimeError):
    pass


_P, _I, _L, _F = C.c_void_p, C.c_int, C.c_int64, C.c_float
_PROTOS = {
    "i2v_create": ([_I, C.POINTER(_P)], _I),
    "i2v_destroy": ([_P], _I),
    "i2v_last_error": ([], C.c_char_p),
    "i2v_abi_version": ([], _I),
    "i2v_backend": ([], C.c_char_p),
    "i2v_backend_stat": ([C.c_char_p], C.c_longlong),
    "i2v_net_create": ([_P, C.POINTER(_I)], _I),
    "i2v_net_destroy": ([_P, _I], _I),
    "i2v_net_add_buffer": ([_P, _I, _I, _I, _I, C.POINTER(_I)], _I),
    "i2v_net_add_tensor": ([_P, _I, _I, _I, _I, _I, C.POINTER(_I)], _I),
    "i2v_net_set_input": ([_P, _I, _I], _I),
    "i2v_net_set_relu_gain": ([_P, _I, _I, _F], _I),
    "i2v_net_add_conv": ([_P, _I, C.POINTER(ConvDesc), _P, _P, _P], _I),
    "i2v_net_add_conv_grouped": ([_P, _I, C.POINTER(ConvDesc), _I, _P, _P, _P], _I),
    "i2v_net_add_conv_depthwise": ([_P, _I, C.POINTER(ConvDesc), _P, _P, _P], _I),
    "i2v_net_add_maxpool": ([_P, _I, C.POINTER(PoolDesc)], _I),
    "i2v_net_add_conv_preact": ([_P, _I, C.POINTER(ConvDesc), _P, _P, _P, _P, _P], _I),
    "i2v_net_add_avgpool": ([_P, _I, C.POINTER(PoolDesc)], _I),
    "i2v_net_add_buffer3d": ([_P, _I, _I, _I, _I, _I, C.POINTER(_I)], _I),
    "i2v_net_add_conv3d": ([_P, _I, C.POINTER(Conv3dDesc), _P, _P, _P], _I),
    "i2v_net_add_maxpool3d": ([_P, _I, C.POINTER(Pool3dDesc)], _I),
    "i2v_net_add_attention": ([_P, _I, C.POINTER(AttnDesc)], _I),
    "i2v_net_add_se": ([_P, _I, C.POINTER(SeDesc), _P, _P, _P, _P], _I),
    "i2v_net_tensor_frames": ([_P, _I, _I, C.POINTER(_I)], _I),
    "i2v_net_plan": ([_P, _I, C.POINTER(_I), _I, _I], _I),
    "i2v_net_workspace_bytes": ([_P, _I], C.c_size_t),
    "i2v_net_fusion_info": ([_P, _I, _P], _I),
    "i2v_net_scpair_info": ([_P, _I, _P], _I),
    "i2v_net_forward": ([_P, _I, _P, _I, _P], _I),
    "i2v_net_hook_info": ([_P, _I, _I, C.POINTER(_P), C.POINTER(_L), C.POINTER(_P), C.POINTER(_L),
                           C.POINTER(_L), C.POINTER(C.c_int32)], _I),
    "i2v_net_backward": ([_P, _I, _P, _I, _P], _I),
    "i2v_net_read_tensor": ([_P, _I, _I, _I, _P, _I, _P], _I),
    "i2v_timing_enable": ([_P, _I], _I),
    "i2v_timing_collect": ([_P, C.POINTER(C.c_double), C.POINTER(C.c_double), C.POINTER(_L), _I], _I),
    "i2v_timing_collect_ex": ([_P, C.POINTER(C.c_double), _I, _I], _I),
    "i2v_clip_from_u8_f32": ([_P, _P, _I, _I, _I, _I, _P], _I),
    "i2v_clip_resize_crop_u8_f32": ([_P, _P, _P, _P, _I, _I, _I, _I, _I, _I, _I, _I, _I, _I, _P], _I),
    "i2v_frames_from_video_f32": ([_P, _P, _P, _I, _I, _I, _I, _P], _I),
    "i2v_compose_f32": ([_P, _P, _P, _I, _I, _I, _I, _F, _I, _P], _I),
    "i2v_cossim_scratch_bytes": ([_L, _I], C.c_size_t),
    "i2v_cossim_fwd_bwd_f32": ([_P, _L, _P, _L, _L, _I, _P, _I, _F, _I, _I, _P, _P, _L, _P, _P], _I),
    "i2v_std_fwd_bwd_f32": ([_P, _L, _L, _I, _I, _I, _P, _P, _L, _P, _P], _I),
    "i2v_std_reduce_f32": ([_P, _L, _L, _I, _P, _P], _I),
    "i2v_std_grad_f32": ([_P, _L, _L, _I, _L, _I, _I, _P, _P, _L, _P, _P], _I),
    "i2v_adam_step_f32": ([_P, _P, _P, _P, _P, _L, _I, _F, C.c_double, C.c_double, C.c_double, C.c_double, _I, _P], _I),
    "i2v_sign_step_f32": ([_P, _P, _P, _L, _L, _F, _F, _P], _I),
    "i2v_sign_step_delta_f32": ([_P, _P, _L, _F, _P], _I),
    "i2v_sign_step_delta_gx_f32": ([_P, _P, _P, _L, _F, _F, _P], _I),
    "i2v_ilaf_reduce_f32": ([_P, _L, _P, _P, _L, _I, _P, _P], _I),
    "i2v_ilaf_grad_f32": ([_P, _L, _P, _P, _L, _I, C.c_double, _I, _I, _P, _P, _L, _P, _P], _I),
    "i2v_ilaf_scratch_bytes": ([_L, _I, _I], C.c_size_t),
    "i2v_ilaf_reduce_seg_f32": ([_P, _L, _P, _P, _L, _I, _I, _P, _P], _I),
    "i2v_ilaf_grad_seg_f32": ([_P, _L, _P, _P, _L, _I, _I, _P, _I, _I, _P, _P, _L, _P, _P], _I),
    "i2v_tap_distance_f32": ([_P, _L, _P, _L, _I, _I, C.c_double, _I, _I, _P, _P, _L, _P, _P], _I),
    "i2v_head_scratch_bytes": ([_I, _I], C.c_size_t),
    "i2v_head_ce_f32": ([_P, _L, _I, _I, _I, _I, _P, _P, _I, _P, _F, _I, _I, _P, _P, _P, _L, _P, _P], _I),
    "i2v_clip_resample_crop_u8_f32": ([_P, _P, _P, _P, _I, _P, _P, _I, _I, _I, _I, _I, _I, _I, _I, _I, _I, _I, _P], _I),
    "i2v_tt_grad_mix_f32": ([_P, _P, _P, _P, _I, _L, _I, _I, _F, _P], _I),
    "i2v_resample_nearest_f32": ([_P, _P, _L, _I, _I, _I, _I, _P, _P, _P], _I),
    "i2v_resample_nearest_bwd_f32": ([_P, _P, _L, _I, _I, _I, _I, _P, _P, _P, _P, _P], _I),
    "i2v_dwconv1d_f32": ([_P, _P, _L, _I, _L, _P, _I, _P], _I),
    "i2v_tap_scratch_bytes": ([_L], _L),
    "i2v_tap_perts_f32": ([_P, _P, _P, _I, _I, _I, _I, _I, _P], _I),
    "i2v_tap_sign_abs_f32": ([_P, _P, _P, _L, _P, _P], _I),
    "i2v_tap_grad_f32": ([_P, _P, _P, _I, _I, _I, _I, _I, _F, _P], _I),
    "i2v_grad_post_scratch_bytes": ([_I, _I, _I, _I, _I, _I], _L),
    "i2v_grad_post_f32": ([_P, _P, _P, _I, _I, _I, _I, _I, _I, _I, _F, _P, _P], _I),
    "i2v_head_pool_f32": ([_P, _L, _I, _I, _I, _I, _I, _I, _P, _P], _I),
    "i2v_head_logits_ce_f32": ([_I, _I, _P, _P, _I, _P, _F, _P, _P, _P, _P], _I),
    "i2v_head_grad_f32": ([_P, _L, _I, _I, _I, _I, _I, _I, _I, _I, _P, _L, _P, _P], _I),
    "i2v_aens_coeffs_f32": ([_P, _P, _F, _I, _P], _I),
    "i2v_aens_reduce_f32": ([_P, _P, _I, _I, _P, _P, _P], _I),
}
EXPORTS = tuple(_PROTOS)
_LOADER_PROTOS = {
    "i2v_clip_gather_scratch_bytes": ([_I, _I, _I, _I], _L),
    "i2v_clip_gather_resize_crop_u8_f32": ([_P, _L, _P, _P, _I, _I, _P, _I, _P, _I, _I, _I, _P, _P, _L, _P], _I),
}
LOADER_EXPORTS = tuple(_LOADER_PROTOS)


class VitConfig(C.Structure):
    _fields_ = [(n, C.c_int32) for n in ("img", "patch", "in_chans", "dim", "heads", "mlp", "blocks")] + [("ln_eps", C.c_float)]


_VIT_PROTOS = {
    "i2v_vit_create": ([_I, C.POINTER(VitConfig), C.POINTER(_P), _I, C.POINTER(C.c_int32), _I, _I, C.POINTER(_P)], _I),
    "i2v_vit_create_ex": ([_I, C.POINTER(VitConfig), _I, C.POINTER(_P), _I, C.POINTER(C.c_int32), _I, _I, C.POINTER(_P)], _I),
    "i2v_vit_destroy": ([_P], _I),
    "i2v_vit_workspace_bytes": ([_P], _L),
    "i2v_vit_forward": ([_P, _P, _I, _P], _I),
    "i2v_vit_backward": ([_P, _P, _I, _P], _I),
    "i2v_vit_hook_info": ([_P, _I, C.POINTER(_P), C.POINTER(_L), C.POINTER(_P), C.POINTER(_L), C.POINTER(_L)], _I),
    "i2v_vit_read_hook": ([_P, _I, _I, _P, _I, _P], _I),
    "i2v_vit_linear_f32": ([_P, _I, _I, _P, _P, _I, _P, _P, _P, _P], _I),
    "i2v_vit_linear_bwd_f32": ([_P, _I, _I, _P, _I, _P, _P, _P], _I),
    "i2v_vit_layernorm_f32": ([_P, _L, _I, _P, _P, _F, _P, _P, _P, _P], _I),
    "i2v_vit_layernorm_bwd_f32": ([_P, _P, _P, _P, _P, _L, _I, _P, _P, _P, _P], _I),
    "i2v_vit_probs_ld": ([_I], _I),
    "i2v_vit_attention_f32": ([_P, _I, _I, _I, _I, _F, _P, _P, _P], _I),
    "i2v_vit_attention_bwd_f32": ([_P, _P, _P, _I, _I, _I, _I, _F, _P, _P, _P], _I),
    "i2v_vit_embed_f32": ([_P, _I, _I, _I, _I, _P, _P, _P, _P, _I, _P, _P, _P, _P], _I),
    "i2v_vit_embed_bwd_f32": ([_P, _I, _I, _I, _I, _P, _I, _P, _P, _I, _P], _I),
    "i2v_vit_embed_ex_f32": ([_P, _I, _I, _I, _I, _P, _P, _P, _I, _P, _I, _P, _P, _P, _P], _I),
    "i2v_vit_embed_bwd_ex_f32": ([_P, _I, _I, _I, _I, _P, _I, _I, _P, _P, _I, _P], _I),
}
VIT_EXPORTS = tuple(_VIT_PROTOS)


class SwinConfig(C.Structure):
# ... 92 lines not shown
```

### include/i2v_hip.h

```cpp
#ifndef I2V_HIP_H
#define I2V_HIP_H
#include <stddef.h>
#include <stdint.h>

#ifdef __cplusplus
extern "C" {
#endif

typedef struct i2v_ctx* i2v_handle;

int i2v_create(int device, i2v_handle* out);
int i2v_destroy(i2v_handle h);
const char* i2v_last_error(void);
int i2v_abi_version(void);
const char* i2v_backend(void);
long long i2v_backend_stat(const char* name);

typedef struct {
    int32_t src, dst;
    int32_t cin, cout, kh, kw, stride, pad;
    int32_t relu;
    int32_t residual;
} i2v_conv_desc;

typedef struct {
    int32_t src, dst;
    int32_t k, stride, pad;
} i2v_pool_desc;

int i2v_net_create(i2v_handle h, int* net);
int i2v_net_destroy(i2v_handle h, int net);
int i2v_net_add_buffer(i2v_handle h, int net, int C, int H, int W, int* buf);
int i2v_net_add_tensor(i2v_handle h, int net, int buf, int c_off, int C, int post_relu, int* tensor);
int i2v_net_set_input(i2v_handle h, int net, int tensor);
int i2v_net_set_relu_gain(i2v_handle h, int net, int tensor, float gain);
int i2v_net_add_conv(i2v_handle h, int net, const i2v_conv_desc* d, const float* weight,
                     const float* scale, const float* shift);
int i2v_net_add_conv_grouped(i2v_handle h, int net, const i2v_conv_desc* d, int groups, const float* weight,
                             const float* scale, const float* shift);
int i2v_net_add_conv_depthwise(i2v_handle h, int net, const i2v_conv_desc* d, const float* weight,
                               const float* scale, const float* shift);
int i2v_net_add_maxpool(i2v_handle h, int net, const i2v_pool_desc* d);
int i2v_net_add_conv_preact(i2v_handle h, int net, const i2v_conv_desc* d, const float* weight,
                            const float* scale, const float* shift, const float* pre_scale,
                            const float* pre_shift);
int i2v_net_add_avgpool(i2v_handle h, int net, const i2v_pool_desc* d);
typedef struct {
    int32_t src, dst;
    int32_t cin, cout, kt, kh, kw;
    int32_t stride_t, stride, pad_t, pad, dil_t;
    int32_t relu, residual;
} i2v_conv3d_desc;
typedef struct {
    int32_t src, dst;
    int32_t kt, k, stride_t, stride, pad_t, pad;
} i2v_pool3d_desc;
int i2v_net_add_buffer3d(i2v_handle h, int net, int C, int T, int H, int W, int* buf);
int i2v_net_add_conv3d(i2v_handle h, int net, const i2v_conv3d_desc* d, const float* weight,
                       const float* scale, const float* shift);
int i2v_net_add_maxpool3d(i2v_handle h, int net, const i2v_pool3d_desc* d);
typedef struct {
    int32_t theta, phi, g, dst;
    float scale;
} i2v_attn_desc;
int i2v_net_add_attention(i2v_handle h, int net, const i2v_attn_desc* d);
typedef struct {
    int32_t src, dst, residual;
    int32_t C, rd, relu;
} i2v_se_desc;
int i2v_net_add_se(i2v_handle h, int net, const i2v_se_desc* d, const float* W1, const float* b1, const float* W2, const float* b2);
int i2v_net_tensor_frames(i2v_handle h, int net, int tensor, int* T);
int i2v_net_plan(i2v_handle h, int net, const int* hook_tensors, int n_hooks, int max_frames);
size_t i2v_net_workspace_bytes(i2v_handle h, int net);
int i2v_net_fusion_info(i2v_handle h, int net, int32_t out[4]);
int i2v_net_scpair_info(i2v_handle h, int net, int32_t out[4]);

int i2v_net_forward(i2v_handle h, int net, const float* x, int frames, void* stream);
int i2v_net_hook_info(i2v_handle h, int net, int hook, float** act, int64_t* act_stride,
                      float** grad, int64_t* grad_stride, int64_t* D, int32_t* post_relu);
int i2v_net_backward(i2v_handle h, int net, float* gx, int accumulate, void* stream);
int i2v_net_read_tensor(i2v_handle h, int net, int tensor, int which, float* out, int frames,
                        void* stream);

int i2v_timing_enable(i2v_handle h, int enable);
int i2v_timing_collect(i2v_handle h, double* ms_by_kind, double* flops_by_kind,
                       int64_t* launches_by_kind, int n_kinds);
int i2v_timing_collect_ex(i2v_handle h, double* out, int n_kinds, int n_fields);

int i2v_clip_from_u8_f32(const uint8_t* frames, float* video, int b, int t, int h, int w, void* stream);
int i2v_clip_resize_crop_u8_f32(const uint8_t* frames, float* video, const int32_t* xtab, const int32_t* ytab, int b, int t,
                                int H, int W, int rh, int rw, int crop_y, int crop_x, int out_h, int out_w, void* stream);
int i2v_clip_resample_crop_u8_f32(const uint8_t* frames, float* video, const int32_t* xbounds, const int32_t* xcoef, int kx,
                                  const int32_t* ybounds, const int32_t* ycoef, int ky, int b, int t, int H, int W, int rh, int rw,
                                  int crop_y, int crop_x, int out_h, int out_w, void* stream);
int i2v_frames_from_video_f32(const float* video, float* x, float* u, int b, int f, int h, int w,
                              void* stream);
int i2v_compose_f32(const float* u, const float* delta, float* x, int b, int f, int h, int w,
                    float eps, int video_layout, void* stream);
size_t i2v_cossim_scratch_bytes(int64_t D, int frames);
int i2v_cossim_fwd_bwd_f32(const float* a, int64_t a_stride, const float* b, int64_t b_stride,
                           int64_t D, int frames, const float* coef_dev, int coef_index,
                           float coef_host, int mask_relu, int accumulate, float* cos_out,
                           float* grad, int64_t grad_stride, void* scratch, void* stream);
int i2v_std_fwd_bwd_f32(const float* a, int64_t a_stride, int64_t D, int frames, int mask_relu,
                        int accumulate, float* std_out, float* grad, int64_t grad_stride,
                        void* scratch, void* stream);
int i2v_std_reduce_f32(const float* a, int64_t a_stride, int64_t D, int frames, void* scratch, void* stream);
int i2v_std_grad_f32(const float* a, int64_t a_stride, int64_t D, int frames, int64_t total_count,
                     int mask_relu, int accumulate, float* std_out, float* grad, int64_t grad_stride,
                     void* scratch, void* stream);
int i2v_adam_step_f32(float* delta, float* m, float* v, const float* gx, const float* u,
                      int64_t frames, int hw, float eps, double lr, double beta1, double beta2,
                      double adam_eps, int step_t, void* stream);
int i2v_sign_step_f32(float* adv, const float* u, const float* grad, int64_t n, int64_t chan_stride,
                      float step, float eps, void* stream);
int i2v_sign_step_delta_f32(float* delta, const float* grad, int64_t n, float step, void* stream);
int i2v_sign_step_delta_gx_f32(float* delta, const float* gx, const float* u, int64_t n, float eps,
                               float step, void* stream);
int i2v_ilaf_reduce_f32(const float* a, int64_t a_stride, const float* ori, const float* adv0, int64_t D,
                        int frames, void* scratch, void* stream);
int i2v_ilaf_grad_f32(const float* a, int64_t a_stride, const float* ori, const float* adv0, int64_t D,
                      int frames, double init_norm, int mask_relu, int accumulate, float* loss_out,
                      float* grad, int64_t grad_stride, void* scratch, void* stream);
size_t i2v_ilaf_scratch_bytes(int64_t D, int frames, int frames_per_seg);
int i2v_ilaf_reduce_seg_f32(const float* a, int64_t a_stride, const float* ori, const float* adv0, int64_t D,
                            int frames, int frames_per_seg, void* scratch, void* stream);
int i2v_ilaf_grad_seg_f32(const float* a, int64_t a_stride, const float* ori, const float* adv0, int64_t D,
                          int frames, int frames_per_seg, const double* init_sq, int mask_relu, int accumulate,
                          float* loss_out, float* grad, int64_t grad_stride, void* scratch, void* stream);
int i2v_tap_distance_f32(const float* a, int64_t a_stride, const float* clean, int64_t D, int frames, int frames_per_seg,
                         double coef, int mask_relu, int accumulate, float* dist_out, float* grad, int64_t grad_stride,
                         void* scratch, void* stream);
size_t i2v_head_scratch_bytes(int C, int clips);
int i2v_head_ce_f32(const float* a, int64_t a_stride, int C, int HW, int T, int clips, const float* W, const float* bias,
                    int K, const int32_t* labels, float scale, int mask_relu, int accumulate, float* logits, float* loss_each,
                    float* grad, int64_t grad_stride, void* scratch, void* stream);
int i2v_head_pool_f32(const float* a, int64_t a_stride, int C, int HW, int T, int clips, int Ctot, int c_off, void* scratch, void* stream);
int i2v_head_logits_ce_f32(int Ctot, int clips, const float* W, const float* bias, int K, const int32_t* labels, float scale,
                           float* logits, float* loss_each, void* scratch, void* stream);
int i2v_head_grad_f32(const float* a, int64_t a_stride, int C, int HW, int T, int clips, int Ctot, int c_off, int mask_relu,
                      int accumulate, float* grad, int64_t grad_stride, void* scratch, void* stream);
int i2v_tt_grad_mix_f32(const float* grads, float* out, const float* kernel, const int32_t* moves, int D, int64_t NC, int T, int HW,
                        float weight, void* stream);
int i2v_resample_nearest_f32(const float* src, float* dst, int64_t planes, int Hs, int Ws, int Hd, int Wd, const int32_t* map_y,
                             const int32_t* map_x, void* stream);
int i2v_resample_nearest_bwd_f32(const float* g, float* gsrc, int64_t planes, int Hd, int Wd, int Hs, int Ws, const int32_t* ylo,
                                 const int32_t* yhi, const int32_t* xlo, const int32_t* xhi, void* stream);
int i2v_dwconv1d_f32(const float* src, float* dst, int64_t outer, int len, int64_t inner, const float* taps, int k, void* stream);
int64_t i2v_grad_post_scratch_bytes(int b, int c, int f, int h, int w, int mode);
int i2v_grad_post_f32(const float* g, float* momentum, float* out, int b, int c, int f, int h, int w, int frame_major, int mode, float decay,
                      void* scratch, void* stream);
int64_t i2v_tap_scratch_bytes(int64_t n);
int i2v_tap_perts_f32(const float* adv, const float* videos, float* out, int b, int c, int f, int h, int w, void* stream);
int i2v_tap_sign_abs_f32(const float* smooth, float* sign_out, float* reg, int64_t n, void* scratch, void* stream);
int i2v_tap_grad_f32(const float* gx, const float* boxsign, float* out, int b, int c, int f, int h, int w, float weight, void* stream);
int i2v_aens_coeffs_f32(const float* prev, float* coeffs, float momentum, int L, void* stream);
int i2v_aens_reduce_f32(const float* cos, const float* coeffs, int L, int frames, float* feat_sum,
                        float* weighted, void* stream);
// ... 6 lines not shown
```

Measured before the change: 755.4.

## Fuse column-parity pairs of stride-2 sub-grid conv launches into one kernel

Adds a paired implicit-GEMM kernel that runs the even-column and odd-column phase launches of a stride-2 decomposed convolution (likely the transposed/backward-data conv) in one block. The first result is held in registers and interleaved with the second inside the epilogue, so each output row is written once as full float4s. The goal is to remove one launch and the strided half-writes per pair. The planner admits eligible adjacent launches, and autotuning keeps the pair only where it times faster than running the two separately. The cost is more register pressure from holding the first tile and a narrower set of eligibility conditions.

Measured after the change: 761.1, median of 6. No clear change (+0.8%).

```diff
diff --git a/__graft_entry__.py b/__graft_entry__.py
--- a/__graft_entry__.py
+++ b/__graft_entry__.py
@@ -17,18 +17,19 @@
 
 ENGINE_UNITS = ["i2v_engine.cpp", "i2v_pack.cpp", "i2v_plan.cpp", "i2v_tune.cpp", "i2v_run.cpp", "i2v_loop_api.cpp"]
 UNITS = ["i2v_kernels.hip", "i2v_conv_cfg0.hip", "i2v_conv_cfg1.hip", "i2v_conv_cfg2.hip", "i2v_conv_cfg3.hip", "i2v_conv_cfg4.hip",
-         "i2v_conv_cfg5.hip", "i2v_conv_scpair.hip", "i2v_conv_stems.hip", "i2v_fastblock.hip", "i2v_gconv.hip", "i2v_dwconv.hip", "i2v_se.hip", "i2v_loader.hip", "i2v_vit.hip", "i2v_vit.cpp", "i2v_swin.hip", "i2v_swin.cpp",
+         "i2v_conv_cfg5.hip", "i2v_conv_scpair.hip", "i2v_conv_s2pair.hip", "i2v_conv_stems.hip", "i2v_fastblock.hip", "i2v_gconv.hip", "i2v_dwconv.hip", "i2v_se.hip", "i2v_loader.hip", "i2v_vit.hip", "i2v_vit.cpp", "i2v_swin.hip", "i2v_swin.cpp",
          "i2v_convnext.hip", "i2v_convnext.cpp", "i2v_mixer.hip", "i2v_mixer.cpp",
          ] + ENGINE_UNITS
 HEADERS = ["i2v_kernels.h", "i2v_params.h", "i2v_be.h", "i2v_conv_tile.h", "i2v_conv_launch.h", "i2v_vit_kernels.h", "i2v_swin_kernels.h", "i2v_xf.h",
            "i2v_net.h", "i2v_se_host.h", "i2v_convnext_host.h", "i2v_xf_host.h", "i2v_hip_stub.h",
-           "i2v_mixer_host.h", "i2v_gelu.h", "i2v_scpair_host.h"]
+           "i2v_mixer_host.h", "i2v_gelu.h", "i2v_scpair_host.h", "i2v_s2pair_host.h"]
 FLAGS = ["--offload-arch=gfx950", "-O3", "-ffp-contract=off", "-std=c++20", "-fPIC", "-DI2V_SEPARATE_UNITS",
          "-DI2V_HAVE_GCONV", "-DI2V_HAVE_DWCONV",
          "-DI2V_HAVE_SE",
          "-DI2V_HAVE_CONVNEXT",
          "-DI2V_HAVE_MIXER",
-         "-DI2V_HAVE_SCPAIR"]
+         "-DI2V_HAVE_SCPAIR",
+         "-DI2V_HAVE_S2PAIR"]
 
 
 def build_lib(experimental: bool = False) -> str:
@@ -62,7 +63,7 @@
 
 def build() -> None:
     build_lib(experimental=False)
-    deps = [os.path.join(CSRC, f) for f in ENGINE_UNITS + ["i2v_net.h", "i2v_kernels.h", "i2v_params.h", "i2v_se_host.h", "i2v_convnext_host.h", "i2v_convnext.cpp", "i2v_mixer_host.h", "i2v_mixer.cpp", "i2v_scpair_host.h", "i2v_gelu.h", "i2v_xf.h", "i2v_xf_host.h", "i2v_hip_stub.h",
+    deps = [os.path.join(CSRC, f) for f in ENGINE_UNITS + ["i2v_net.h", "i2v_kernels.h", "i2v_params.h", "i2v_se_host.h", "i2v_convnext_host.h", "i2v_convnext.cpp", "i2v_mixer_host.h", "i2v_mixer.cpp", "i2v_scpair_host.h", "i2v_s2pair_host.h", "i2v_gelu.h", "i2v_xf.h", "i2v_xf_host.h", "i2v_hip_stub.h",
                                                                "i2v_vit_kernels.h", "i2v_swin_kernels.h"]] + [os.path.join(ROOT, "include", "i2v_hip.h")]
     hs = os.path.join(ROOT, "tests", "hostsim")
     if _stale(os.path.join(hs, "libi2v_hostsim.so"), deps + [os.path.join(hs, "hostsim_backend.cpp")]):
diff --git a/image-to-video-i2v-attack_amd/csrc/i2v_be.h b/image-to-video-i2v-attack_amd/csrc/i2v_be.h
--- a/image-to-video-i2v-attack_amd/csrc/i2v_be.h
+++ b/image-to-video-i2v-attack_amd/csrc/i2v_be.h
@@ -19,7 +19,7 @@
 int hip_fail(hipError_t e, const char* what);
 #define HIPCHK(x) do { hipError_t e_ = (x); if (e_ != hipSuccess) return hip_fail(e_, #x); } while (0)
 #define LAUNCH_CHECK(name) do { hipError_t e_ = hipGetLastError(); if (e_ != hipSuccess) return hip_fail(e_, name); } while (0)
-extern long long g_stat_conv, g_stat_pws, g_stat_bf3, g_stat_igh, g_stat_sth, g_stat_fastblock, g_stat_vfma, g_stat_igv, g_stat_gconv, g_stat_dwconv, g_stat_se, g_stat_cndw, g_stat_mixtok, g_stat_scpair;
+extern long long g_stat_conv, g_stat_pws, g_stat_bf3, g_stat_igh, g_stat_sth, g_stat_fastblock, g_stat_vfma, g_stat_igv, g_stat_gconv, g_stat_dwconv, g_stat_se, g_stat_cndw, g_stat_mixtok, g_stat_scpair, g_stat_s2pair;
 
 __device__ __forceinline__ unsigned fastdiv(unsigned n, unsigned m, unsigned s) {
     return (unsigned)(((unsigned long long)n * m) >> s);
diff --git a/image-to-video-i2v-attack_amd/csrc/i2v_conv_s2pair.hip b/image-to-video-i2v-attack_amd/csrc/i2v_conv_s2pair.hip
--- /dev/null
+++ b/image-to-video-i2v-attack_amd/csrc/i2v_conv_s2pair.hip
@@ -0,0 +1,54 @@
+#include "i2v_conv_tile.h"
+
+#ifndef I2V_S2PAIR_WPE
+#define I2V_S2PAIR_WPE I2V_SMALL_WPE
+#endif
+
+__global__ void __launch_bounds__(256) __attribute__((amdgpu_waves_per_eu(I2V_S2PAIR_WPE, I2V_S2PAIR_WPE)))
+conv_igemm_s2pair(const I2VConvParams a, const I2VConvParams b, const int n_cd_tiles) {
+    constexpr int BD = 64, BP = 64, WD = 2, WP = 2, FR = 32;
+    __shared__ __attribute__((aligned(16))) float smem[conv_lds_floats<BD, BP, WD, false>()];
+    I2V_PROBE_T probe;
+    probe.entry();
+    const int lid = conv_xcd_lid(blockIdx.x, gridDim.x);
+    const int cd0 = (lid % n_cd_tiles) * BD;
+    const int64_t px0 = (int64_t)(lid / n_cd_tiles) * BP;
+
+    constexpr int C4 = BP / 4, RSTEP = 1024 / BP, NQ = WD * FR / RSTEP;
+    float4 ya[NQ];
+    float4 nopre[1]; unsigned nogw[1];
+    {
+        f32x16 acc[1][1];
+        conv_tile_loop<BD, BP, WD, WP, 2, false>(a, cd0, px0, gridDim.x, smem, probe, blockIdx.x, I2V_PRIO_LEVELS, acc, nopre, nogw);
+        float (*Cs)[BP] = reinterpret_cast<float (*)[BP]>(smem);
+        conv_acc_to_rows<BP, WP, false>(acc[0], Cs);
+        const int t = threadIdx.x, c4 = t % C4, rbase = t / C4;
+#pragma unroll
+        for (int q = 0; q < NQ; ++q) ya[q] = *reinterpret_cast<const float4*>(&Cs[rbase + q * RSTEP][c4 * 4]);
+        __syncthreads();
+    }
+    f32x16 acc[1][1];
+    conv_tile_loop<BD, BP, WD, WP, 2, false>(b, cd0, px0, gridDim.x, smem, probe, blockIdx.x, I2V_PRIO_LEVELS, acc, nopre, nogw);
+    conv_vec_epilogue<BD, BP, WD, WP, false, false, false, true>(b, acc, cd0, px0, smem, ya, nullptr, nullptr);
+    probe.exit(blockIdx.x);
+}
+
+long long g_stat_s2pair = 0;
+
+int k_conv_s2pair_ok(const I2VConvParams& a, const I2VConvParams& b) { return i2v_conv_s2pair_ok(a, b) ? 1 : 0; }
+
+int k_conv_s2pair(const I2VConvParams& a_in, const I2VConvParams& b_in, i2v_stream_t s) {
+    I2VConvParams a = a_in, b = b_in;
+    if (!i2v_conv_s2pair_ok(a, b)) { snprintf(g_be_err, sizeof g_be_err, "column-parity pair launch: the two launches do not form a pair"); g_be_has_err = true; return 1; }
+    const int64_t P = (int64_t)b.N * b.Hg * b.Wg;
+    if (P + 1024 >= (1ll << 31)) { snprintf(g_be_err, sizeof g_be_err, "conv launch of more than 2^31 grid pixels"); g_be_has_err = true; return 1; }
+    conv_magics(a); conv_magics(b);
+    const int n_cd = (b.Cd + 63) / 64;
+    const int64_t grid = (P + 63) / 64 * n_cd;
+    if (grid <= 0) return 0;
+    if (grid > 0x7fffffff) { snprintf(g_be_err, sizeof g_be_err, "conv grid too large"); g_be_has_err = true; return 1; }
+    __atomic_fetch_add(&g_stat_s2pair, 1, __ATOMIC_RELAXED);
+    hipLaunchKernelGGL(conv_igemm_s2pair, dim3((unsigned)grid), dim3(256), 0, (hipStream_t)s, a, b, n_cd);
+    LAUNCH_CHECK("conv_s2pair");
+    return 0;
+}
diff --git a/image-to-video-i2v-attack_amd/csrc/i2v_conv_tile.h b/image-to-video-i2v-attack_amd/csrc/i2v_conv_tile.h
--- a/image-to-video-i2v-attack_amd/csrc/i2v_conv_tile.h
+++ b/image-to-video-i2v-attack_amd/csrc/i2v_conv_tile.h
@@ -56,7 +56,7 @@
     return stage > epi ? stage : epi;
 }
 
-template <int BD, int BP, int WD, bool PREF, bool MF16, bool FUSE, typename PT>
+template <int BD, int BP, int WD, bool PREF, bool MF16, bool FUSE, bool S2 = false, typename PT>
 __device__ __forceinline__ void conv_vec_rows(const PT& p, const int i, const int cd0, const int64_t px0, const float (*const Cs)[BP], const int t,
                                               const float4* const pre0, const unsigned* const pregw, float* const mid) {
     constexpr int FR = MF16 ? 16 : 32;
@@ -75,15 +75,32 @@
     const bool pok = pp < P;
     const int64_t n = pok ? fastdiv((unsigned)pp, p.dv_hw_m, p.dv_hw_s) : 0;
     const int64_t poff = pp - n * HWg;
+    static_assert(!S2 || (!PREF && !MF16 && !FUSE), "column-parity pair: the plain dense row pass");
+    constexpr int NH = S2 ? 2 : 1;
+    int64_t hoff0 = 0, hoff1 = 0; bool hok0 = false, hok1 = false;
+    if constexpr (S2) {
+        const int rem = (int)poff;
+        const int gi0 = (int)fastdiv((unsigned)rem, p.dv_w_m, p.dv_w_s), gi1 = (int)fastdiv((unsigned)(rem + 2), p.dv_w_m, p.dv_w_s);
+        const int oh0 = gi0 * 2 + p.oh0, oh1 = gi1 * 2 + p.oh0;
+        hoff0 = (int64_t)oh0 * p.Wo + 2 * (rem - gi0 * p.Wg); hok0 = oh0 < p.Ho;
+        hoff1 = (int64_t)oh1 * p.Wo + 2 * (rem + 2 - gi1 * p.Wg); hok1 = oh1 < p.Ho;
+    }
+    float4 vb = make_float4(0.f, 0.f, 0.f, 0.f);
+    (void)vb; (void)hoff0; (void)hoff1; (void)hok0; (void)hok1;
     #pragma unroll
-    for (int q = 0; q < NQ; ++q) {
+    for (int qh = 0; qh < NQ * NH; ++qh) {
+        const int q = qh / NH, h = qh % NH;
         const int row = rbase + q * RSTEP;
         const int cd = cd0 + (row / FR) * (BD / WD) + i * FR + (row % FR);
-        const bool valid = pok && cd < p.Cd;
+        const bool valid = S2 ? pok && cd < p.Cd && (h ? hok1 : hok0) : pok && cd < p.Cd;
         float4 v = make_float4(0.f, 0.f, 0.f, 0.f);
         if (valid) {
-        v = *reinterpret_cast<const float4*>(&Cs[row][c4 * 4]);
-        const int64_t o = (int64_t)cd * HoWo + poff;
+        if constexpr (S2) {
+            if (h == 0 || !hok0) vb = *reinterpret_cast<const float4*>(&Cs[row][c4 * 4]);
+            const float4 va = pre0[q];
+            v = h ? make_float4(va.z, vb.z, va.w, vb.w) : make_float4(va.x, vb.x, va.y, vb.y);
+        } else v = *reinterpret_cast<const float4*>(&Cs[row][c4 * 4]);
+        const int64_t o = (int64_t)cd * HoWo + (S2 ? (h ? hoff1 : hoff0) : poff);
         if (p.gate_scale) {
             const float4 m = *reinterpret_cast<const float4*>(p.mask + n * p.mask_nstride + o);
             const float gs = p.gate_scale[cd], gt = p.gate_shift[cd];
@@ -114,8 +131,9 @@
         }
         if (p.relu) { v.x = fmaxf(v.x, 0.f); v.y = fmaxf(v.y, 0.f); v.z = fmaxf(v.z, 0.f); v.w = fmaxf(v.w, 0.f); }
         if (p.gate) {
-            const unsigned w = PREF ? pregw[q] : p.gate[(int64_t)cd * p.gate_stride + ((p.gate_pix0 + pp) >> 5)];
-            const unsigned g = w >> ((unsigned)(p.gate_pix0 + pp) & 31u);
+            const int64_t gbit = S2 ? p.gate_pix0 + n * HoWo + (h ? hoff1 : hoff0) : p.gate_pix0 + pp;
+            const unsigned w = PREF ? pregw[q] : p.gate[(int64_t)cd * p.gate_stride + (gbit >> 5)];
+            const unsigned g = w >> ((unsigned)gbit & 31u);
             if (!(g & 1u)) v.x = 0.f;
             if (!(g & 2u)) v.y = 0.f;
             if (!(g & 4u)) v.z = 0.f;
@@ -135,7 +153,7 @@
         }
         if constexpr (FUSE)
             *reinterpret_cast<float4*>(mid + (cd - cd0) * BP + c4 * 4) = v;
-        if (p.gate_out) {
+        if (!S2 && p.gate_out) {
             unsigned nib = valid ? ((v.x > 0.f ? 1u : 0u) | (v.y > 0.f ? 2u : 0u) | (v.z > 0.f ? 4u : 0u) | (v.w > 0.f ? 8u : 0u)) : 0u;
             nib <<= 4 * (lane & 7);
             nib |= (unsigned)__builtin_amdgcn_update_dpp(0, (int)nib, 0xB1, 0xF, 0xF, true);
@@ -162,7 +180,7 @@
             Cs[wd * FR + I2V_FROW(r)][wpx * (BP / WP) + j * FR + l31] = acc[j][r];
     __syncthreads();
 }
-template <int BD, int BP, int WD, int WP, bool PREF, bool MF16, bool FUSE, typename ACC, typename PT>
+template <int BD, int BP, int WD, int WP, bool PREF, bool MF16, bool FUSE, bool S2 = false, typename ACC, typename PT>
 __device__ __forceinline__ void conv_vec_epilogue(const PT& p, ACC (&acc)[BD / WD / (MF16 ? 16 : 32)][BP / WP / (MF16 ? 16 : 32)], const int cd0,
                                                   const int64_t px0, float* const smem, const float4* const pre0, const unsigned* const pregw,
                                                   float* const mid) {
@@ -172,7 +190,7 @@
 #pragma unroll
     for (int i = 0; i < TD; ++i) {
         conv_acc_to_rows<BP, WP, MF16>(acc[i], Cs);
-        conv_vec_rows<BD, BP, WD, PREF, MF16, FUSE>(p, i, cd0, px0, Cs, t, pre0, pregw, mid);
+        conv_vec_rows<BD, BP, WD, PREF, MF16, FUSE, S2>(p, i, cd0, px0, Cs, t, pre0, pregw, mid);
     }
 }
 #undef I2V_FROW
diff --git a/image-to-video-i2v-attack_amd/csrc/i2v_engine.cpp b/image-to-video-i2v-attack_amd/csrc/i2v_engine.cpp
--- a/image-to-video-i2v-attack_amd/csrc/i2v_engine.cpp
+++ b/image-to-video-i2v-attack_amd/csrc/i2v_engine.cpp
@@ -449,6 +449,15 @@
     return 0;
 }
 
+extern "C" int i2v_net_s2pair_info(i2v_handle h, int net, int32_t out[2]) {
+    Net* n = get_net(h, net); if (!n) return 1;
+    if (!n->planned || !out) return fail("i2v_net_s2pair_info: net not planned");
+    out[0] = out[1] = 0;
+    for (const std::vector<Launch>* L : {&n->fwd, &n->bwd})
+        for (const Launch& l : *L) { out[0] += l.s2_ok ? 1 : 0; out[1] += (l.s2_ok && l.s2_b[0]) ? 1 : 0; }
+    return 0;
+}
+
 extern "C" size_t i2v_net_workspace_bytes(i2v_handle h, int net) {
     Net* n = get_net(h, net); if (!n) return 0;
     return n->arena_floats * sizeof(float) + n->weight_bytes;
diff --git a/image-to-video-i2v-attack_amd/csrc/i2v_kernels.h b/image-to-video-i2v-attack_amd/csrc/i2v_kernels.h
--- a/image-to-video-i2v-attack_amd/csrc/i2v_kernels.h
+++ b/image-to-video-i2v-attack_amd/csrc/i2v_kernels.h
@@ -52,6 +52,24 @@
 }
 int k_conv_scpair_ok(const I2VConvParams& a, const I2VConvParams& b);
 int k_conv_scpair(const I2VConvParams& a, const I2VConvParams& b, i2v_stream_t s);
+inline bool i2v_conv_s2pair_ok(const I2VConvParams& a, const I2VConvParams& b) {
+    for (const I2VConvParams* q : {&a, &b}) {
+        if (!q->tap_uniform || q->pointwise || q->temporal || q->quad || q->pre_scale || q->gate_scale || q->mask || q->gate_out || q->bf3 ||
+            q->blk > 1 || q->blkt > 1) return false;
+        if (q->osh != 2 || q->osw != 2 || (q->add0 && q->add0_stride != 1)) return false;
+    }
+    if (a.ow0 != 0 || b.ow0 != 1 || a.oh0 != b.oh0 || a.oh0 < 0 || a.oh0 > 1) return false;
+    if (a.N != b.N || a.Hg != b.Hg || a.Wg != b.Wg || a.Cd != b.Cd || a.Ho != b.Ho || a.Wo != b.Wo) return false;
+    if (a.src != b.src || a.src_nstride != b.src_nstride || a.Cs != b.Cs || a.Hs != b.Hs || a.Ws != b.Ws) return false;
+    if (!a.dst || a.dst != b.dst || a.dst_nstride != b.dst_nstride) return false;
+    if (a.shift != b.shift || a.relu != b.relu || a.add0 != b.add0 || a.add0_nstride != b.add0_nstride || a.add1 != b.add1 || a.add1_nstride != b.add1_nstride ||
+        a.gate != b.gate || a.gate_stride != b.gate_stride || a.gate_pix0 != b.gate_pix0) return false;
+    if (a.Hg <= 0 || a.Wg % 2 != 0 || (a.Hg * a.Wg) % 4 != 0 || a.Wo != 2 * a.Wg || a.Wo % 4 != 0 || (a.Ho * a.Wo) % 4 != 0 || 2 * (a.Hg - 1) + a.oh0 >= a.Ho) return false;
+    if (a.dst_nstride % 4 != 0 || (a.add0 && a.add0_nstride % 4 != 0) || (a.add1 && a.add1_nstride % 4 != 0) || (a.gate && a.gate_pix0 % 4 != 0)) return false;
+    return (((uintptr_t)a.dst | (uintptr_t)a.add0 | (uintptr_t)a.add1) & 15) == 0;
+}
+int k_conv_s2pair_ok(const I2VConvParams& a, const I2VConvParams& b);
+int k_conv_s2pair(const I2VConvParams& a, const I2VConvParams& b, i2v_stream_t s);
 int k_conv_candidates(const I2VConvParams& p, int* out);
 inline int i2v_fastblock_rows(const I2VConvParams& a, const I2VConvParams& b, const I2VConvParams* c, const I2VConvParams* d) {
     auto plain = [](const I2VConvParams& q) {
diff --git a/image-to-video-i2v-attack_amd/csrc/i2v_kernels.hip b/image-to-video-i2v-attack_amd/csrc/i2v_kernels.hip
--- a/image-to-video-i2v-attack_amd/csrc/i2v_kernels.hip
+++ b/image-to-video-i2v-attack_amd/csrc/i2v_kernels.hip
@@ -26,6 +26,7 @@
     if (!strcmp(name, "convnext_dw_launches")) return __atomic_load_n(&g_stat_cndw, __ATOMIC_RELAXED);
     if (!strcmp(name, "mixer_tokens_launches")) return __atomic_load_n(&g_stat_mixtok, __ATOMIC_RELAXED);
     if (!strcmp(name, "scpair_launches")) return __atomic_load_n(&g_stat_scpair, __ATOMIC_RELAXED);
+    if (!strcmp(name, "s2pair_launches")) return __atomic_load_n(&g_stat_s2pair, __ATOMIC_RELAXED);
 #ifdef I2V_EXPERIMENTAL
     if (!strcmp(name, "experimental")) return 1;
 #else
diff --git a/image-to-video-i2v-attack_amd/csrc/i2v_net.h b/image-to-video-i2v-attack_amd/csrc/i2v_net.h
--- a/image-to-video-i2v-attack_amd/csrc/i2v_net.h
+++ b/image-to-video-i2v-attack_amd/csrc/i2v_net.h
@@ -93,6 +93,8 @@
     int fb_b[4] = {0, 0, 0, 0};
     int sc_ok = 0;
     int sc_b[4] = {0, 0, 0, 0};
+    int s2_ok = 0;
+    int s2_b[4] = {0, 0, 0, 0};
     bool sc_private = false;
     int ov_after = -2, ov_join = -1;
 };
@@ -175,6 +177,8 @@
 bool sc_pair_ok(const Launch& a, const Launch& b);
 bool sc_fits(const Launch& a, const Launch& b, int frames);
 int sc_run(const Launch& a, const Launch& b, int frames, i2v_stream_t s);
+bool s2_pair_ok(const Launch& a, const Launch& b);
+int s2_run(const Launch& a, const Launch& b, int frames, i2v_stream_t s);
 extern long long g_overlap_launches;
 
 #pragma GCC visibility pop
diff --git a/image-to-video-i2v-attack_amd/csrc/i2v_run.cpp b/image-to-video-i2v-attack_amd/csrc/i2v_run.cpp
--- a/image-to-video-i2v-attack_amd/csrc/i2v_run.cpp
+++ b/image-to-video-i2v-attack_amd/csrc/i2v_run.cpp
@@ -4,6 +4,9 @@
 #endif
 #ifndef I2V_HAVE_SCPAIR
 #include "i2v_scpair_host.h"
+#endif
+#ifndef I2V_HAVE_S2PAIR
+#include "i2v_s2pair_host.h"
 #endif
 
 #include <stdio.h>
@@ -78,6 +81,28 @@
     return 0;
 }
 
+bool s2_pair_ok(const Launch& a, const Launch& b) {
+    if (a.kind != L_CONV || b.kind != L_CONV || a.src_is_input || b.src_is_input || a.T != b.T || a.node != b.node) return false;
+    I2VConvParams pa, pb;
+    sc_prep(a, b, a.T, &pa, &pb);
+#ifdef I2V_HAVE_S2PAIR
+    return k_conv_s2pair_ok(pa, pb) != 0;
+#else
+    return s2pair_host::ok(pa, pb) != 0;
+#endif
+}
+int s2_run(const Launch& a, const Launch& b, int frames, i2v_stream_t s) {
+    I2VConvParams pa, pb;
+    sc_prep(a, b, frames, &pa, &pb);
+    pb.cfg = 1 + 3;
+#ifdef I2V_HAVE_S2PAIR
+    CHECK_BE(k_conv_s2pair(pa, pb, s));
+#else
+    if (s2pair_host::run(pa, pb, s)) return fail("column-parity pair: the two launches do not form a pair");
+#endif
+    return 0;
+}
+
 int fast_run(const std::vector<Launch>& L, size_t li, int frames, const float* x, i2v_stream_t s) {
     const int g = L[li].fb_ok;
     I2VConvParams q[4];
@@ -138,9 +163,10 @@
     return t;
 }
 
-static double launch_flops(const std::vector<Launch>& L, size_t li, int fb, int fuse, int sc, int frames, int clips) {
+static double launch_flops(const std::vector<Launch>& L, size_t li, int fb, int fuse, int sc, int s2, int frames, int clips) {
     const Launch& l = L[li];
     double flops = 0.0;
+    if (s2) return launch_flops(L, li, 0, 0, -1, 0, frames, clips) + launch_flops(L, li + 1, 0, 0, -1, 0, frames, clips);
     if (sc >= 0) return 2.0 * frames * l.conv.Hg * l.conv.Wg * ((double)l.conv.Cd * l.conv.K + (double)L[sc].conv.Cd * L[sc].conv.K);
     if (fb) { for (int j = 0; j < fb; ++j) { const Launch& m = L[li + j]; flops += m.alg_flops_per_frame > 0 ? m.alg_flops_per_frame * frames : 2.0 * frames * m.conv.Hg * m.conv.Wg * (double)m.conv.Cd * m.conv.K; } }
     else if ((l.kind == L_CONV || l.kind == L_GCONV || l.kind == L_DWCONV) && l.alg_flops_per_frame > 0) flops = l.alg_flops_per_frame * frames;
@@ -163,9 +189,12 @@
     return 4;
 }
 
-static double launch_bytes(const std::vector<Launch>& L, size_t li, int fb, int fuse, int sc, int frames, int clips, int accumulate) {
+static double launch_bytes(const std::vector<Launch>& L, size_t li, int fb, int fuse, int sc, int s2, int frames, int clips, int accumulate) {
     const Launch& l = L[li];
     const I2VConvParams& q = l.conv;
+    if (s2)
+        return launch_bytes(L, li, 0, 0, -1, 0, frames, clips, accumulate) + launch_bytes(L, li + 1, 0, 0, -1, 0, frames, clips, accumulate) -
+               4.0 * clips * q.Ts * q.Cs * q.Hs * q.Ws;
     const double out = (double)frames * q.Hg * q.Wg * q.Cd;
     const double src = (double)clips * q.Ts * q.Cs * q.Hs * q.Ws;
     double b = 4.0 * (src + (double)q.K * q.Cd + out);
@@ -209,10 +238,10 @@
     TimedLaunch* prev = nullptr;
     TimedLaunch* seg = nullptr;
 
-    TimedLaunch* open(const std::vector<Launch>& L, size_t li, int fb, int fuse, int sc, int frames, int clips, int accumulate) {
+    TimedLaunch* open(const std::vector<Launch>& L, size_t li, int fb, int fuse, int sc, int s2, int frames, int clips, int accumulate) {
         const Launch& l = L[li];
         const int kind = launch_timing_kind(l, backward_pass);
-        const double flops = launch_flops(L, li, fb, fuse, sc, frames, clips);
+        const double flops = launch_flops(L, li, fb, fuse, sc, s2, frames, clips);
         const bool conv = l.kind == L_CONV || l.kind == L_IMGGRAD || l.kind == L_GCONV || l.kind == L_DWCONV;
         if (h->timing == 2) {
             if (!seg || seg->kind != kind) {
@@ -220,13 +249,13 @@
                 seg = timing_begin(h, kind, 0.0, s, seg);
                 if (seg) seg->count = 0;
             }
-            if (seg) { seg->flops += flops; seg->count += 1; if (conv) seg->bytes += launch_bytes(L, li, fb, fuse, sc, frames, clips, accumulate); else seg->bytes += l.se_bytes_per_frame * frames; }
+            if (seg) { seg->flops += flops; seg->count += 1; if (conv) seg->bytes += launch_bytes(L, li, fb, fuse, sc, s2, frames, clips, accumulate); else seg->bytes += l.se_bytes_per_frame * frames; }
             return prev = nullptr;
         }
         TimedLaunch* const tl = prev = timing_begin(h, kind, flops, s, prev);
         if (tl && conv) {
             tl->Cd = l.conv.Cd; tl->K = l.conv.K; tl->HWg = l.conv.Hg * l.conv.Wg; tl->frames = frames; tl->pw = l.conv.pointwise;
-            tl->bytes = launch_bytes(L, li, fb, fuse, sc, frames, clips, accumulate);
+            tl->bytes = launch_bytes(L, li, fb, fuse, sc, s2, frames, clips, accumulate);
         }
         if (tl && l.kind == L_AGEMM) {
             const I2VAttnGemm& q = l.ag;
@@ -291,7 +320,7 @@
     const bool overlap = !h->timing && n.side && !side.at.empty() && in_frames <= n.ov_max_frames;
     if (overlap) n.ov_used = 0;
     if (overlap && side.issue(-1)) return 1;
-    auto leads_group = [&](size_t k) { return L[k].kind == L_CONV && ((L[k].fuse_ok && L[k].fuse_b[bucket]) || (L[k].fb_ok && L[k].fb_b[bucket])); };
+    auto leads_group = [&](size_t k) { return L[k].kind == L_CONV && ((L[k].fuse_ok && L[k].fuse_b[bucket]) || (L[k].fb_ok && L[k].fb_b[bucket]) || (L[k].s2_ok && L[k].s2_b[bucket])); };
     int sc_from = -1; size_t sc_at = 0;
     for (size_t li = 0; li < L.size(); ++li) {
         Launch& l = L[li];
@@ -309,8 +338,10 @@
         const int fuse = (l.kind == L_CONV && l.fuse_ok && li + 1 < L.size() && frames * l.conv.Hg * l.conv.Wg > 0 && fused_fits(l, L[li + 1], frames))
                              ? l.fuse_b[bucket] : 0;
         const int fb = (l.kind == L_CONV && l.fb_ok && li + l.fb_ok <= L.size() && frames * l.conv.Hg * l.conv.Wg > 0) ? l.fb_b[bucket] * l.fb_ok : 0;
+        const int s2 = (l.kind == L_CONV && l.s2_ok && !overlap && sc < 0 && li + 1 < L.size() && frames * l.conv.Hg * l.conv.Wg > 0 && fused_fits(l, L[li + 1], frames))
+                           ? l.s2_b[bucket] : 0;
         if (overlap && side.join((int)li + (fb ? fb - 1 : fuse ? 1 : 0))) return 1;
-        TimedLaunch* const tl = h->timing ? timing.open(L, li, fb, fuse, sc, frames, clips, accumulate) : nullptr;
+        TimedLaunch* const tl = h->timing ? timing.open(L, li, fb, fuse, sc, s2, frames, clips, accumulate) : nullptr;
         struct Stop { TimedLaunch* t; i2v_stream_t s; ~Stop() { if (t) be_event_record(t->stop, s); } } stop{tl, s};
         switch (l.kind) {
             case L_CONV:
@@ -322,6 +353,7 @@
                     break;
                 }
                 if (fuse) { if (fused_run(l, L[li + 1], frames, x, fuse == 2, s)) return 1; ++li; break; }
+                if (s2) { if (s2_run(l, L[li + 1], frames, s)) return 1; ++li; break; }
                 if (fb) {
                     const int rc = fast_run(L, li, frames, x, s);
                     if (rc == 1) return 1;
diff --git a/image-to-video-i2v-attack_amd/csrc/i2v_s2pair_host.h b/image-to-video-i2v-attack_amd/csrc/i2v_s2pair_host.h
--- /dev/null
+++ b/image-to-video-i2v-attack_amd/csrc/i2v_s2pair_host.h
@@ -0,0 +1,15 @@
+#pragma once
+#include "i2v_kernels.h"
+
+namespace eng {
+namespace s2pair_host {
+
+inline int ok(const I2VConvParams& a, const I2VConvParams& b) { return i2v_conv_s2pair_ok(a, b) ? 1 : 0; }
+
+inline int run(const I2VConvParams& a, const I2VConvParams& b, i2v_stream_t s) {
+    if (!i2v_conv_s2pair_ok(a, b)) return 1;
+    return (k_conv(a, s) || k_conv(b, s)) ? 1 : 0;
+}
+
+}
+}
diff --git a/image-to-video-i2v-attack_amd/csrc/i2v_tune.cpp b/image-to-video-i2v-attack_amd/csrc/i2v_tune.cpp
--- a/image-to-video-i2v-attack_amd/csrc/i2v_tune.cpp
+++ b/image-to-video-i2v-attack_amd/csrc/i2v_tune.cpp
@@ -186,6 +186,21 @@
                                 a.conv.K, b.conv.K, b.conv.Cd, b.conv.Hg, b.conv.Wg, (int)other, (int)dep);
                     break;
                 }
+            }
+        }
+    }
+    {
+        const bool s2_off = [] { const char* e = getenv("I2V_S2PAIR"); return e && e[0] == '0'; }();
+        for (std::vector<Launch>* L : {&n.fwd, &n.bwd}) {
+            for (Launch& l : *L) { l.s2_ok = 0; for (int bk = 0; bk < 4; ++bk) l.s2_b[bk] = 0; }
+            for (size_t i = 0; !s2_off && i + 1 < L->size(); ++i) {
+                Launch& a = (*L)[i]; const Launch& b = (*L)[i + 1];
+                if (a.sc_ok || a.fuse_ok || a.fb_ok || b.sc_ok || b.fuse_ok || b.fb_ok || !s2_pair_ok(a, b)) continue;
+                a.s2_ok = 1; for (int bk = 0; bk < 4; ++bk) a.s2_b[bk] = 1;
+                if (getenv("I2V_FUSE_DEBUG"))
+                    fprintf(stderr, "[i2v s2pair] %s launches %zu + %zu admitted (K %d + %d -> Cd %d, class grid %dx%d, row parity %d)\n", L == &n.fwd ? "fwd" : "bwd", i, i + 1,
+                            a.conv.K, b.conv.K, a.conv.Cd, a.conv.Hg, a.conv.Wg, a.conv.oh0);
+                ++i;
             }
         }
     }
@@ -267,7 +282,7 @@
         for (int i = 0; i < M; ++i) {
             const Launch& l = (*L)[i];
             for (int j = 0; j < l.fb_ok && i + j < M; ++j) member[i + j] = 1;
-            if (l.fuse_ok) { member[i] = 1; if (i + 1 < M) member[i + 1] = 1; }
+            if (l.fuse_ok || l.s2_ok) { member[i] = 1; if (i + 1 < M) member[i + 1] = 1; }
         }
         n.ov_at[k].assign(M + 1, {});
         int hoisted = 0;
@@ -466,6 +481,33 @@
     return 0;
 }
 
+int tune_s2pairs(Net& n, Probe& pr, int max_clips) {
+    for (std::vector<Launch>* L : {&n.fwd, &n.bwd})
+        for (size_t i = 0; i + 1 < L->size(); ++i) {
+            Launch& a = (*L)[i];
+            if (!a.s2_ok) continue;
+            Launch& b = (*L)[i + 1];
+            const int rc = for_each_bucket(max_clips, a.conv.Tg, [&](int bk, int lf) -> int {
+                if (lf * a.conv.Hg * a.conv.Wg == 0 || !fused_fits(a, b, lf)) return 0;
+                const int ca = a.conv.cfg, cb = b.conv.cfg;
+                if (a.cfg_b[bk]) a.conv.cfg = a.cfg_b[bk];
+                if (b.cfg_b[bk]) b.conv.cfg = b.cfg_b[bk];
+                float t_sep = 0.f, t_pair = 0.f;
+                const int rc = pr.time([&] { return conv_run(a, lf, pr.x, pr.gx, 0, nullptr) || conv_run(b, lf, pr.x, pr.gx, 0, nullptr); }, 3, &t_sep) ||
+                               pr.time([&] { return s2_run(a, b, lf, nullptr); }, 3, &t_pair);
+                a.conv.cfg = ca; b.conv.cfg = cb;
+                if (rc) return 1;
+                a.s2_b[bk] = t_pair < t_sep ? 1 : 0;
+                if (getenv("I2V_FUSE_DEBUG"))
+                    fprintf(stderr, "[i2v s2pair] %s launches %zu + %zu (K %d + %d -> Cd %d, class grid %dx%d) at %d frames: separate %.1f us, pair %.1f us -> %s\n",
+                            list_name(n, L), i, i + 1, a.conv.K, b.conv.K, a.conv.Cd, a.conv.Hg, a.conv.Wg, lf, 1e3f * t_sep, 1e3f * t_pair, a.s2_b[bk] ? "pair" : "separate");
+                return 0;
+            });
+            if (rc) return 1;
+        }
+    return 0;
+}
+
 }
 
 int autotune(Net& n) {
@@ -480,6 +522,7 @@
         rc = tune_tiles(n, pr, max_clips);
         if (!rc && on_device) rc = tune_fastblocks(n, pr, max_clips);
         if (!rc && on_device) rc = tune_scpairs(n, pr, max_clips);
+        if (!rc && on_device) rc = tune_s2pairs(n, pr, max_clips);
         static const bool fuse_on = [] { const char* e = getenv("I2V_FUSE"); return e && e[0] == '1'; }();
         if (!rc && fuse_on && on_device) rc = tune_pairs(n, pr, max_clips);
     }
diff --git a/image-to-video-i2v-attack_amd/i2v_amd/engine.py b/image-to-video-i2v-attack_amd/i2v_amd/engine.py
--- a/image-to-video-i2v-attack_amd/i2v_amd/engine.py
+++ b/image-to-video-i2v-attack_amd/i2v_amd/engine.py
@@ -423,6 +423,11 @@
         _lib.check(self.eng.capi, self.eng.capi.i2v_net_scpair_info(self.eng.h, self.id, out))
         return tuple(int(v) for v in out)
 
+    def s2pair_info(self):
+        out = (C.c_int32 * 2)()
+        _lib.check(self.eng.capi, self.eng.capi.i2v_net_s2pair_info(self.eng.h, self.id, out))
+        return tuple(int(v) for v in out)
+
     def forward(self, x: torch.Tensor):
         _lib.check(self.eng.capi, self.eng.capi.i2v_net_forward(self.eng.h, self.id, _ptr(x, self.eng), x.shape[0], self.eng.stream()))
 
diff --git a/image-to-video-i2v-attack_amd/i2v_amd/lib.py b/image-to-video-i2v-attack_amd/i2v_amd/lib.py
--- a/image-to-video-i2v-attack_amd/i2v_amd/lib.py
+++ b/image-to-video-i2v-attack_amd/i2v_amd/lib.py
@@ -67,6 +67,7 @@
     "i2v_net_workspace_bytes": ([_P, _I], C.c_size_t),
     "i2v_net_fusion_info": ([_P, _I, _P], _I),
     "i2v_net_scpair_info": ([_P, _I, _P], _I),
+    "i2v_net_s2pair_info": ([_P, _I, _P], _I),
     "i2v_net_forward": ([_P, _I, _P, _I, _P], _I),
     "i2v_net_hook_info": ([_P, _I, _I, C.POINTER(_P), C.POINTER(_L), C.POINTER(_P), C.POINTER(_L),
                            C.POINTER(_L), C.POINTER(C.c_int32)], _I),
diff --git a/include/i2v_hip.h b/include/i2v_hip.h
--- a/include/i2v_hip.h
+++ b/include/i2v_hip.h
@@ -74,6 +74,7 @@
 size_t i2v_net_workspace_bytes(i2v_handle h, int net);
 int i2v_net_fusion_info(i2v_handle h, int net, int32_t out[4]);
 int i2v_net_scpair_info(i2v_handle h, int net, int32_t out[4]);
+int i2v_net_s2pair_info(i2v_handle h, int net, int32_t out[2]);
 
 int i2v_net_forward(i2v_handle h, int net, const float* x, int frames, void* stream);
 int i2v_net_hook_info(i2v_handle h, int net, int hook, float** act, int64_t* act_stride,
```
